# richarddurbin/hash10x

Measured on AMD Instinct MI355X. Metric: read-pairs/s through --readFQB + --hashDepthRange + --cluster (mosh construction + per-barcode clustering), higher is better.
Workload: dtype u64; 1 GPU; yeast-like-2.5M; read_pairs=2500000, barcodes=10000, B=24, k=21, w=31, clusterThreshold=5, parallelism=single GPU

## Files before the change

### hash10x_amd/csrc/common.hpp

```cpp
#pragma once
#include <hip/hip_runtime.h>
#include <cstdint>
#include <cstdio>
#include <cstdarg>
#include <cstring>
#include <cstdlib>
#include <ctime>
#include <string>
#include <vector>
#include <map>
#include <mutex>
#include "../../include/h10x.h"

namespace h10x {

constexpr int WAVE = 64;
typedef unsigned long long u64;
typedef uint32_t u32;
typedef uint16_t u16;
typedef uint8_t  u8;

static_assert(sizeof(h10x_block) == 32, "ClusterBlock layout (hash10x.c:62-70)");
static_assert(sizeof(h10x_clushash) == 8, "ClusterHash layout (hash10x.c:35-43)");

// ... 53 lines not shown
    if (!count) count = 1;
    size_t bytes = (count * sizeof(T) + 255) & ~(size_t)255;
    dev = AllocScope::device(); st = AllocScope::stream();
    hipError_t e = hipSuccess;
    void *q = DevCache::disabled() ? nullptr : DevCache::take(dev, st, bytes, cap);
    if (!q) {
      static const bool log = getenv("H10X_ALLOC_LOG") != nullptr;
      timespec t0, t1; if (log) clock_gettime(CLOCK_MONOTONIC, &t0);
      cap = bytes; e = hipMalloc(&q, bytes);
      if (e != hipSuccess && !DevCache::disabled()) { DevCache::trim(dev); e = hipMalloc(&q, bytes); }
      if (e == hipSuccess) { __atomic_fetch_add(&DevCache::freshCalls(), 1, __ATOMIC_RELAXED); __atomic_fetch_add(&DevCache::freshBytes(), (unsigned long long)bytes, __ATOMIC_RELAXED); }
      if (log) { clock_gettime(CLOCK_MONOTONIC, &t1); fprintf(stderr, "h10x alloc: %.1f MB fresh, %.3f ms\n", bytes / 1e6, (t1.tv_sec - t0.tv_sec) * 1e3 + (t1.tv_nsec - t0.tv_nsec) / 1e6); }
    }
    if (e == hipSuccess) { p = (T *)q; n = count; } else { p = nullptr; cap = 0; }
    if (e == hipSuccess && DevCache::poison()) (void)hipMemsetAsync(p, 0xA5, bytes, AllocScope::stream());
    return e;
  }
  void swap(DevBuf &o) { std::swap(p, o.p); std::swap(n, o.n); std::swap(cap, o.cap); std::swap(dev, o.dev); std::swap(st, o.st); }
  size_t bytes() const { return n * sizeof(T); }
};

enum TimerId { T_RUNS = 0, T_MOSH, T_FALLBACK, T_COMPACT, T_SORT_HASH, T_RANK, T_PROBE, T_CLUSHASH, T_CSR,
               T_GOOD, T_CLUSTER, T_CLUSTER_K, T_CLUSTER_MAIN, T_SPLIT, T_COUNT };
static const char *const kTimerNames[T_COUNT] = {
  "block_runs", "mosh_extract", "mosh_fallback", "compact_entries", "sort_by_hash", "index_rank",
  "probe_table", "clushash_build", "csr_build", "good_hashes", "cluster", "cluster_kernel", "cluster_main", "cluster_split" };

struct Timer { hipEvent_t a = nullptr, b = nullptr; double ms = 0; uint64_t launches = 0; bool pending = false; };

enum XchgId { X_HOST_COUNTS = 0, X_ENTRIES, X_FIRST_COUNTS, X_INDEX_BACK, X_INDEX_DEPTH, X_LIST_HEADS, X_LIST_DATA, X_TABLES, X_OWNER_LISTS, X_GATHER, X_COUNT };
static const char *const kXchgNames[X_COUNT] = {
  "host_counts (small host allgathers: sizes, counts)", "entries_to_hash_owners (all-to-all)", "first_seen_counts (allgather)", "indices_back (all-to-all)",
  "index_depth (allgather)", "list_heads (allgather: index + length of the in-range hashes)", "list_data (allgather: the in-range barcode lists)",
  "hash_tables (allgather: hashValue, for --writeHash / the crib)", "owner_lists_rebuild (after --clusterSplit)", "gather_to_rank0" };
struct XchgStat { u64 calls = 0, bytesOut = 0, bytesIn = 0, maxPeerOut = 0; Timer t, tIn; int beside = -1; };

constexpr size_t ROWS_PAD = 128;
constexpr int MAX_SEGS = 8;
struct BlockSeg { u32 localStart, count, globalBase; };
struct SegMap {
  int n; BlockSeg s[MAX_SEGS];
  __host__ __device__ u32 globalOf(u32 l) const {
    for (int k = n - 1; k > 0; --k) if (l >= s[k].localStart) return s[k].globalBase + (l - s[k].localStart);
    return s[0].globalBase + l;
  }
};
struct ShardSegInfo { u32 rank, localStart, count, globalBase; u64 entries; };

struct Ctx {
  h10x_params prm{};
  u64 keyInv = 1; int keyShift = 0; int keyBits = 64;
  bool wantPacked = false; int entCodeBits = 0;
  int device = 0;
  hipStream_t stream = nullptr;
  hipStream_t aux[3] = {nullptr, nullptr, nullptr};
  hipEvent_t evFork = nullptr, evJoin[3] = {nullptr, nullptr, nullptr};
  int numCU = 256;
  bool ownStream = false;
  std::string err;

  DevBuf<u32> hashIndex;
  DevBuf<u64> hashValue;
  DevBuf<u32> hashDepth;
  DevBuf<u64> rowStart;
  DevBuf<u32> rows;
  DevBuf<h10x_block> blocks;
  DevBuf<u64> blockOff;
  DevBuf<h10x_clushash> clusHash;
  u32 hashNumber = 1, nBlocks = 0;
  u32 maxBlockHashes = 0xFFFFFFFFu;
  u64 nEntries = 0, nRecords = 0;
  bool haveState = false;

  DevBuf<u8>  within;
  DevBuf<u16> goodPos;
  DevBuf<u32> nGood;
  DevBuf<u64> goodRow;
  DevBuf<u32> goodEntries;
  DevBuf<u32> clusterRaw;
  bool haveRange = false, haveGood = false; int rangeMin = 0, rangeMax = 0;
  u32 rangeHiMax = 0;
  u32 depthBound = 0xFFFFFFFFu;
  u32 maxGoodDepth = 0, maxGood = 0, meanGood = 0;

  DevBuf<u32> cribCount[2];
  DevBuf<u64> cribFirst[2];
  DevBuf<int16_t> cribChr; DevBuf<u16> cribPos; DevBuf<u8> cribType;
  DevBuf<u32> cribHist;
  u32 cribHistDim = 0; int cribGenomes = 0; bool haveCrib = false;

  struct Comm *comm = nullptr; bool sharded = false;
  u32 codeBase = 0, nBlocksGlobal = 0;
  SegMap segs{1, {{0, 0, 0}}};
  std::vector<ShardSegInfo> allSegs;
  u64 nEntriesGlobal = 0, nRecordsGlobal = 0;
  int rowShift = 0;
  bool ownerListsStale = false;
  DevBuf<u32> oRows, oSegStart, oIndex; u32 oU = 0; u64 oM = 0;
  DevBuf<u64> oHash;
  bool tablesPending = false;

  int64_t optMaxSlots = 0;
  int64_t optClusterLds = 0;
  int64_t optFirstGlobal = 0;
  int64_t optFirstCap = 0;
  int64_t optClusterThreads0 = 0, optClusterBudget0 = 0;
  int64_t optBigRanks = 0;
  int64_t optPrivTable = 0;
  int64_t optProbedTable = 0;
  int64_t optNoPack = 0;
  int64_t optNarrowFirst = 0;
  int64_t optTrEstDiv = 0;
  int64_t optTrClassT = -1;
  int64_t optTrPacked = -1;
  int64_t optStamps = 0;
  int64_t optChunk = 0;
  int64_t optChunkEof = 1;
  std::vector<u64> mergePoints; bool replayDone = false;
  int64_t optRowShift = -1;
  int64_t optReplySort = 0;
  int64_t optOverlap = 1;
  int64_t optOwnerCut = 0;
  int64_t optDeltaLists = -1;
  int64_t optRowsFakeBase = 0;
  int64_t optNbBudget = 0;
  u64 nbStats[4] = {0, 0, 0, 0};
  DevBuf<u32> ingestBuf; u64 ingestRecords = 0, ingestCap = 0; bool ingestAsync = false;
  static constexpr int INGEST_SLOTS = 8; hipEvent_t ingestEv[INGEST_SLOTS] = {};
  int64_t optFaultInject = 0;
  int faultAt(int region) { if (optFaultInject != region) return 0; optFaultInject = 0; return fail("injected fault in fork/join region %d", region); }
  bool timing = false;
  u32 *startFlags = nullptr;
  Timer timers[T_COUNT];
  XchgStat xs[X_COUNT];
  h10x_counters ctr{};

  int fail(const char *fmt, ...) {
    char buf[1024]; va_list ap; va_start(ap, fmt); vsnprintf(buf, sizeof buf, fmt, ap); va_end(ap);
    err = buf; return -1;
  }
  static constexpr size_t MAIL_BYTES = 4096, MAIL_ITEMS = 12;
  unsigned char *mail = nullptr; size_t mailUsed = 0; u32 mailSeq = 0; bool mailDirect = false;
  struct PendingRead { void *dst; const void *dev; size_t off, n; };
  std::vector<PendingRead> pendingReads;
  int readback(void *dst, const void *dev, size_t n) {
    if (!mail) {
      if (hipHostMalloc((void **)&mail, MAIL_BYTES + 64, hipHostMallocCoherent | hipHostMallocMapped) != hipSuccess) { mail = nullptr; return fail("hipHostMalloc of the read-back mailbox failed"); }
      memset(mail, 0, MAIL_BYTES + 64);
    }
    const size_t off = mailUsed, step = (n + 7) & ~(size_t)7;
    if (off + step > MAIL_BYTES || pendingReads.size() >= MAIL_ITEMS) {
      mailDirect = true;
      return hipMemcpyAsync(dst, dev, n, hipMemcpyDeviceToHost, stream) == hipSuccess ? 0 : fail("hipMemcpyAsync (device to host) failed");
    }
    mailUsed += step; pendingReads.push_back(PendingRead{dst, dev, off, n});
    return 0;
  }
  int syncReadbacks();
  int forkStreams(int n) {
    if (!evFork) {
      if (hipEventCreateWithFlags(&evFork, hipEventDisableTiming) != hipSuccess) return fail("hipEventCreate failed");
      for (int i = 0; i < 3; ++i) {
        if (hipStreamCreateWithFlags(&aux[i], hipStreamNonBlocking) != hipSuccess) return fail("hipStreamCreate failed");
        if (hipEventCreateWithFlags(&evJoin[i], hipEventDisableTiming) != hipSuccess) return fail("hipEventCreate failed");
      }
    }
// ... 179 lines not shown
```

### hash10x_amd/csrc/h10x_api.hip

```cpp
#include "common.hpp"
#include "comm.hpp"
#include "build_id.h"
#include <cstdlib>
#include <ctime>
#include <new>
#include <stdexcept>

using namespace h10x;

static int enter(Ctx &c) {
  if (hipSetDevice(c.device) != hipSuccess) return c.fail("hipSetDevice(%d) failed", c.device);
  AllocScope::stream() = c.stream; AllocScope::device() = c.device;
  DevCache::noteStream(c.device, c.stream);
  c.pendingReads.clear(); c.mailUsed = 0; c.mailDirect = false;
  c.stageReset();
  return 0;
}

struct h10x_ctx { Ctx c; };

extern "C" {

int h10x_abi_version(void) { return H10X_ABI_VERSION; }
const char *h10x_build_id(void) { return H10X_BUILD_ID; }
// ... 112 lines not shown
  if (!rm || !set) return -1;
  return rsGuard(M(set), [&] { return stageI_load(reinterpret_cast<RefMap **>(rm), M(set), index, offset, id, depth, rev, loc, max, nIds); });
}
void h10x_refmap_destroy(h10x_refmap *rm) { stageI_destroy(RM(rm)); }
const char *h10x_refmap_error(const h10x_refmap *rm) { return stageI_error(reinterpret_cast<const RefMap *>(rm)); }
int h10x_refmap_info(const h10x_refmap *rm, h10x_refmap_info_t *out) { if (!rm || !out) return -1; stageI_info(reinterpret_cast<const RefMap *>(rm), out); return 0; }
int h10x_refmap_add(h10x_refmap *rm, const uint8_t *codes, const uint64_t *seqStart, uint32_t nSeq, uint32_t idBase, uint64_t *nHits) {
  return rm ? rsGuard(stageI_set(RM(rm)), [&] { return stageI_add(RM(rm), codes, (const u64 *)seqStart, nSeq, idBase, (u64 *)nHits); }) : -1;
}
int h10x_refmap_pack(h10x_refmap *rm, uint32_t *n1, uint32_t *n2, uint32_t *nM) {
  return rm ? rsGuard(stageI_set(RM(rm)), [&] { return stageI_pack(RM(rm), n1, n2, nM); }) : -1;
}
int h10x_refmap_export(h10x_refmap *rm, const uint32_t **index, const uint32_t **offset, const uint32_t **id, const uint32_t **depth, const uint32_t **rev, const uint32_t **loc) {
  return rm ? stageI_export(RM(rm), index, offset, id, depth, rev, loc) : -1;
}
int h10x_refmap_query(h10x_refmap *rm, const uint8_t *codes, const uint64_t *seqStart, uint32_t nSeq, int wantSeeds) {
  return rm ? rsGuard(stageI_set(RM(rm)), [&] { return stageI_query(RM(rm), codes, (const u64 *)seqStart, nSeq, wantSeeds); }) : -1;
}
int h10x_refmap_results(h10x_refmap *rm, uint32_t *nQueries, const uint32_t **counts4, const uint64_t **recStart, const h10x_maprec_t **recs, const uint64_t **seedStart,
                        const h10x_mapseed_t **seeds, const uint32_t **seedPos) {
  return rm ? stageI_results(RM(rm), nQueries, counts4, (const u64 **)recStart, recs, (const u64 **)seedStart, seeds, seedPos) : -1;
}

static int create_fail(char *err, int errlen, const char *fmt, ...) {
  if (err && errlen > 0) { va_list ap; va_start(ap, fmt); vsnprintf(err, (size_t)errlen, fmt, ap); va_end(ap); }
  return -1;
}

int h10x_create(h10x_ctx **out, const h10x_params *p, int device, void *stream, char *err, int errlen) {
  if (!out || !p) return create_fail(err, errlen, "h10x_create: null argument");
  *out = nullptr;
  if (p->k <= 0 || p->w <= 0) return create_fail(err, errlen, "k %d, w %d must be > 0; run without args for usage", p->k, p->w);
  if (p->k >= 32) return create_fail(err, errlen, "seqhash k %d must be between 1 and 32\n", p->k);
  if (p->B < 20 || p->B > 30) return create_fail(err, errlen, "hashTableBits %d out of range 20-30", p->B);
  int n = 0;
  if (hipGetDeviceCount(&n) != hipSuccess || n <= 0)
    return create_fail(err, errlen, "no HIP device available: libh10x_hip has no CPU fallback");
  if (device < 0 || device >= n) return create_fail(err, errlen, "HIP device %d out of range 0..%d", device, n - 1);
  if (hipSetDevice(device) != hipSuccess) return create_fail(err, errlen, "hipSetDevice(%d) failed", device);
  static hipDeviceProp_t propCache[64]; static bool propOK[64];
  if (device >= 64) return create_fail(err, errlen, "HIP device %d out of range", device);
  if (!propOK[device]) {
    if (hipGetDeviceProperties(&propCache[device], device) != hipSuccess) return create_fail(err, errlen, "hipGetDeviceProperties failed");
    propOK[device] = true;
  }
  const hipDeviceProp_t &prop = propCache[device];
  if (strncmp(prop.gcnArchName, "gfx950", 6) != 0)
    return create_fail(err, errlen, "device %d is %s: this library is built for gfx950 (MI355X) only", device, prop.gcnArchName);
  h10x_ctx *h = new (std::nothrow) h10x_ctx();
  if (!h) return create_fail(err, errlen, "out of host memory");
  h->c.prm = *p; h->c.device = device; h->c.stream = (hipStream_t)stream; h->c.numCU = prop.multiProcessorCount;
  if (!stream) {
    if (hipStreamCreateWithFlags(&h->c.stream, hipStreamNonBlocking) != hipSuccess) { delete h; return create_fail(err, errlen, "hipStreamCreate failed"); }
    h->c.ownStream = true;
  }
  *out = h;
  return 0;
}

void h10x_destroy(h10x_ctx *h) {
  if (!h) return;
  (void)enter(h->c);
  (void)hipStreamSynchronize(h->c.stream);
  for (auto &t : h->c.timers) { if (t.a) (void)hipEventDestroy(t.a); if (t.b) (void)hipEventDestroy(t.b); }
  for (int i = 0; i < 3; ++i) { if (h->c.aux[i]) { (void)hipStreamSynchronize(h->c.aux[i]); (void)hipStreamDestroy(h->c.aux[i]); } if (h->c.evJoin[i]) (void)hipEventDestroy(h->c.evJoin[i]); }
  if (h->c.evFork) (void)hipEventDestroy(h->c.evFork);
  if (h->c.xStream) { (void)hipStreamSynchronize(h->c.xStream); (void)hipStreamDestroy(h->c.xStream); h->c.xStream = nullptr; }
  if (h->c.evXFork) (void)hipEventDestroy(h->c.evXFork);
  if (h->c.evXDone) (void)hipEventDestroy(h->c.evXDone);
  for (auto &e : h->c.ingestEv) if (e) (void)hipEventDestroy(e);
  if (h->c.startFlags) (void)hipHostFree(h->c.startFlags);
  if (h->c.mail) (void)hipHostFree(h->c.mail);
  hipStream_t own = h->c.ownStream ? h->c.stream : nullptr; const hipStream_t used = h->c.stream; const int dev = h->c.device;
  delete h;
  (void)hipStreamSynchronize(used);
  DevCache::retireStream(dev, used);
  if (own) (void)hipStreamDestroy(own);
}

const char *h10x_last_error(const h10x_ctx *h) { return h ? h->c.err.c_str() : "null context"; }

static void reset_state(Ctx &c) {
  c.haveState = false; c.haveRange = false; c.haveGood = false; c.rangeMin = c.rangeMax = 0; c.depthBound = 0xFFFFFFFFu; c.rangeHiMax = 0;
  c.within.release(); c.goodPos.release(); c.nGood.release(); c.goodEntries.release(); c.goodRow.release();
  c.hashIndex.release(); c.hashValue.release(); c.hashDepth.release(); c.rowStart.release(); c.rows.release();
  c.blocks.release(); c.blockOff.release(); c.clusHash.release(); c.clusterRaw.release();
  c.hashNumber = 1; c.nBlocks = 0; c.nEntries = 0; c.nRecords = 0; c.maxBlockHashes = 0xFFFFFFFFu;
  c.sharded = false; c.codeBase = 0; c.nBlocksGlobal = 0; c.oRows.release(); c.oSegStart.release(); c.oIndex.release(); c.oU = 0; c.oM = 0;
  c.oHash.release(); c.tablesPending = false;
  c.segs.n = 1; c.segs.s[0] = BlockSeg{0, 0, 0}; c.allSegs.clear(); c.nEntriesGlobal = c.nRecordsGlobal = 0; c.rowShift = 0; c.ownerListsStale = false;
  memset(&c.ctr, 0, sizeof c.ctr);
  c.haveCrib = false; c.cribGenomes = 0; c.cribChr.release(); c.cribPos.release(); c.cribType.release(); c.cribHist.release();
  for (int g = 0; g < 2; ++g) { c.cribCount[g].release(); c.cribFirst[g].release(); }
}

int h10x_read_fqb_device(h10x_ctx *h, const uint32_t *dRec, uint64_t n) {
  if (!h) return -1;
  Ctx &c = h->c;
  H10X_TRY(enter(c));
  if (n && !dRec) return c.fail("h10x_read_fqb_device: null records");
  reset_state(c);
  static const bool prof = getenv("H10X_HOSTPROF") != nullptr;
  timespec t0, t1, t2; clock_gettime(CLOCK_MONOTONIC, &t0);
  DevBuf<u64> entHash; DevBuf<u32> entCode, entRead;
  c.wantPacked = !c.optNoPack;
  { const int rcA = stageA_run(&c, dRec, n, entHash, entCode, entRead); c.wantPacked = false; if (rcA) return rcA; }
  c.segs.n = 1; c.segs.s[0] = BlockSeg{0, c.nBlocks, 0};
  clock_gettime(CLOCK_MONOTONIC, &t1);
  H10X_TRY(stageB_run(&c, entHash, entCode, entRead));
  clock_gettime(CLOCK_MONOTONIC, &t2);
  if (prof) fprintf(stderr, "hostprof: stageA %.3f ms, stageB %.3f ms (wall)\n", 1e3 * (t1.tv_sec - t0.tv_sec) + 1e-6 * (t1.tv_nsec - t0.tv_nsec),
                    1e3 * (t2.tv_sec - t1.tv_sec) + 1e-6 * (t2.tv_nsec - t1.tv_nsec));
  return 0;
}

int h10x_read_fqb(h10x_ctx *h, const uint32_t *hostRec, uint64_t n) {
  if (!h) return -1;
  Ctx &c = h->c;
  H10X_TRY(enter(c));
  if (n && !hostRec) return c.fail("h10x_read_fqb: null records");
  DevBuf<u32> d;
  H10X_HIP(&c, d.alloc(n * 30));
  if (n) H10X_HIP(&c, hipMemcpyAsync(d.p, hostRec, n * 120, hipMemcpyHostToDevice, c.stream));
  H10X_HIP(&c, hipStreamSynchronize(c.stream));
  return h10x_read_fqb_device(h, d.p, n);
}

__global__ void block_offsets_kernel(const h10x_block *__restrict__ blocks, u32 nBlocks, u32 *__restrict__ nHash) {
  const u32 i = blockIdx.x * blockDim.x + threadIdx.x;
  if (i <= nBlocks) nHash[i] = (i >= 1 && i < nBlocks) ? blocks[i].nHash : 0;
}

__global__ void validate_entries_kernel(const h10x_clushash *__restrict__ ch, const u64 *__restrict__ blockOff, const h10x_block *__restrict__ blocks, u32 nBlocks,
                                        u32 hashNumber, u32 *__restrict__ bad) {
  for (u32 b = blockIdx.x + 1; b < nBlocks; b += gridDim.x) {
    const u64 e0 = blockOff[b], e1 = blockOff[b + 1]; const u32 nSub = blocks[b].nSubCluster;
    if (threadIdx.x == 0 && nSub > 255) atomicAdd(&bad[2], 1u);
    for (u64 e = e0 + threadIdx.x; e < e1; e += blockDim.x) {
      const h10x_clushash x = ch[e];
      if (x.hash >= hashNumber) atomicAdd(&bad[0], 1u);
      if (x.subCluster > nSub) atomicAdd(&bad[3], 1u);
    }
  }
}
__global__ void validate_table_kernel(const u32 *__restrict__ table, u64 n, u32 hashNumber, u32 *__restrict__ bad) {
  u64 i = (u64)blockIdx.x * blockDim.x + threadIdx.x; const u64 stride = (u64)gridDim.x * blockDim.x;
  u32 mine = 0;
  for (; i < n; i += stride) if (table[i] >= hashNumber) ++mine;
  if (mine) atomicAdd(&bad[1], mine);
}

}

#include "prim.hpp"

extern "C" {

}
namespace h10x { int shard_adoptLoadedState(Ctx *c, Comm *cm, u32 codeBase, u32 nBlocksGlobal); }
static int upload_state(Ctx &c, const uint32_t *hashIndex, uint32_t hashNumber, const uint64_t *hashValue,
                        const uint32_t *hashDepth, const h10x_block *blocks, uint32_t nBlocks, const h10x_clushash *clusHash) {
  if (!hashIndex || !hashValue || !hashDepth || !blocks || nBlocks < 1 || hashNumber < 1) return c.fail("h10x_load_state: bad argument");
  reset_state(c);
  hipStream_t st = c.stream;
  const u64 tableSize = (u64)1 << c.prm.B;
  u64 H = 0;
  u32 maxHash = 0;
// ... 512 lines not shown
```

### hash10x_amd/csrc/prim.hip

```cpp
#include "prim.hpp"
#include <thread>
#include <rocprim/rocprim.hpp>

namespace h10x {

#define PRIM_TWO_PHASE(c, t, CALL)                                                               \
  do { size_t bytes = 0; void *tmp = nullptr;                                                    \
       hipError_t e = (CALL);                                                                    \
       if (e != hipSuccess) return (c)->fail("rocPRIM size query failed: %s", hipGetErrorName(e)); \
       if (bytes > (t).buf.n) { e = (t).buf.alloc(bytes + (bytes >> 2));                         \
         if (e != hipSuccess) return (c)->fail("out of device memory for %zu bytes of sort/scan scratch", bytes); } \
       tmp = (t).buf.p;                                                                          \
       e = (CALL);                                                                               \
       if (e != hipSuccess) return (c)->fail("rocPRIM call failed: %s", hipGetErrorName(e)); } while (0)

int prim_exclusive_scan_u32(Ctx *c, PrimTemp &t, const u32 *in, u32 *out, size_t n) {
  if (!n) return 0;
  PRIM_TWO_PHASE(c, t, rocprim::exclusive_scan(tmp, bytes, in, out, (u32)0, n, rocprim::plus<u32>(), c->stream));
  return 0;
}
struct RunHead {
  const u64 *key; size_t n; int cb;
  __device__ u32 operator()(size_t i) const { return (i < n && (i == 0 || (key[i] >> cb) != (key[i - 1] >> cb))) ? 1u : 0u; }
};
int prim_run_ordinals_u64(Ctx *c, PrimTemp &t, const u64 *key, int cb, u32 *ord, size_t n) {
  auto flags = rocprim::make_transform_iterator(rocprim::counting_iterator<size_t>(0), RunHead{key, n, cb});
  PRIM_TWO_PHASE(c, t, rocprim::exclusive_scan(tmp, bytes, flags, ord, (u32)0, n + 1, rocprim::plus<u32>(), c->stream));
  return 0;
}
int prim_exclusive_scan_u32_u64(Ctx *c, PrimTemp &t, const u32 *in, u64 *out, size_t n) {
  if (!n) return 0;
  auto in64 = rocprim::make_transform_iterator(in, [] __device__(u32 v) -> u64 { return (u64)v; });
  PRIM_TWO_PHASE(c, t, rocprim::exclusive_scan(tmp, bytes, in64, out, (u64)0, n, rocprim::plus<u64>(), c->stream));
  return 0;
}
int prim_inclusive_scan_u32(Ctx *c, PrimTemp &t, const u32 *in, u32 *out, size_t n) {
  if (!n) return 0;
  PRIM_TWO_PHASE(c, t, rocprim::inclusive_scan(tmp, bytes, in, out, n, rocprim::plus<u32>(), c->stream));
  return 0;
}
int prim_sort_pairs_u64_u32(Ctx *c, PrimTemp &t, const u64 *kin, u64 *kout, const u32 *vin, u32 *vout, size_t n, int b0, int b1) {
  if (!n) return 0;
  PRIM_TWO_PHASE(c, t, rocprim::radix_sort_pairs(tmp, bytes, kin, kout, vin, vout, n, (unsigned)b0, (unsigned)b1, c->stream));
  return 0;
}
int prim_sort_pairs_u32_u32(Ctx *c, PrimTemp &t, const u32 *kin, u32 *kout, const u32 *vin, u32 *vout, size_t n, int b0, int b1) {
  if (!n) return 0;
  PRIM_TWO_PHASE(c, t, rocprim::radix_sort_pairs(tmp, bytes, kin, kout, vin, vout, n, (unsigned)b0, (unsigned)b1, c->stream));
  return 0;
}
struct MailArgs { const unsigned char *src[Ctx::MAIL_ITEMS]; u32 off[Ctx::MAIL_ITEMS], n[Ctx::MAIL_ITEMS]; u32 count; };
__global__ void mail_post_kernel(MailArgs a, unsigned char *mail, u32 *flag, u32 seq) {
  for (u32 i = 0; i < a.count; ++i)
    for (u32 b = threadIdx.x; b < a.n[i]; b += blockDim.x) mail[a.off[i] + b] = a.src[i][b];
  __threadfence_system();
  __syncthreads();
  if (threadIdx.x == 0) __hip_atomic_store(flag, seq, __ATOMIC_RELEASE, __HIP_MEMORY_SCOPE_SYSTEM);
}
int Ctx::syncReadbacks() {
  hipError_t e = hipSuccess;
  if (pendingReads.empty() || mailDirect) e = hipStreamSynchronize(stream);
  if (!pendingReads.empty() && e == hipSuccess) {
    MailArgs a; a.count = (u32)pendingReads.size();
    for (u32 i = 0; i < a.count; ++i) { a.src[i] = (const unsigned char *)pendingReads[i].dev; a.off[i] = (u32)pendingReads[i].off; a.n[i] = (u32)pendingReads[i].n; }
    u32 *flag = (u32 *)(mail + MAIL_BYTES);
    const u32 seq = ++mailSeq ? mailSeq : ++mailSeq;
    mail_post_kernel<<<1, 64, 0, stream>>>(a, mail, flag, seq);
    e = hipGetLastError();
    for (u64 spins = 0; e == hipSuccess && __atomic_load_n(flag, __ATOMIC_ACQUIRE) != seq; ++spins) {
#if !defined(__HIP_DEVICE_COMPILE__)
#if defined(__x86_64__) || defined(__i386__)
      __builtin_ia32_pause();
#else
      std::this_thread::yield();
#endif
#endif
      if ((spins & 0xFFF) == 0xFFF) {
        const hipError_t q = hipStreamQuery(stream);
        if (q == hipErrorNotReady) continue;
        if (q == hipSuccess && __atomic_load_n(flag, __ATOMIC_ACQUIRE) == seq) break;
        e = q == hipSuccess ? hipErrorUnknown : q;
      }
    }
    if (e == hipSuccess) for (const PendingRead &r : pendingReads) memcpy(r.dst, mail + r.off, r.n);
  }
  pendingReads.clear(); mailUsed = 0; mailDirect = false;
  return e == hipSuccess ? 0 : fail("HIP error %s at a read-back", hipGetErrorString(e));
}

int prim_sort_pairs_u32_v16(Ctx *c, PrimTemp &t, const u32 *kin, u32 *kout, const Val16 *vin, Val16 *vout, size_t n, int b0, int b1) {
  if (!n) return 0;
  PRIM_TWO_PHASE(c, t, rocprim::radix_sort_pairs(tmp, bytes, kin, kout, vin, vout, n, (unsigned)b0, (unsigned)b1, c->stream));
  return 0;
}
using SortKeys64Config = rocprim::radix_sort_config<rocprim::default_config, rocprim::default_config,
    rocprim::radix_sort_onesweep_config<rocprim::kernel_config<1024, 8>, rocprim::kernel_config<1024, 8>, 8, rocprim::block_radix_rank_algorithm::match>, 1024 * 1024>;
int prim_sort_keys_u64(Ctx *c, PrimTemp &t, const u64 *kin, u64 *kout, size_t n, int b0, int b1) {
  if (!n) return 0;
  PRIM_TWO_PHASE(c, t, rocprim::radix_sort_keys<SortKeys64Config>(tmp, bytes, kin, kout, n, (unsigned)b0, (unsigned)(b1 > 64 ? 64 : b1), c->stream));
  return 0;
}
int prim_seg_sort_keys_u64(Ctx *c, PrimTemp &t, const u64 *kin, u64 *kout, u32 n, u32 nSeg, const u32 *begin, const u32 *end, int b0, int b1) {
  if (!n || !nSeg) return 0;
  PRIM_TWO_PHASE(c, t, rocprim::segmented_radix_sort_keys(tmp, bytes, kin, kout, n, nSeg, begin, end, (unsigned)b0, (unsigned)b1, c->stream));
  return 0;
}
int prim_seg_sort_keys_u32(Ctx *c, PrimTemp &t, const u32 *kin, u32 *kout, u32 n, u32 nSeg, const u32 *begin, const u32 *end, int b0, int b1) {
  if (!n || !nSeg) return 0;
  PRIM_TWO_PHASE(c, t, rocprim::segmented_radix_sort_keys(tmp, bytes, kin, kout, n, nSeg, begin, end, (unsigned)b0, (unsigned)b1, c->stream));
  return 0;
// ... 16 lines not shown
```

### hash10x_amd/csrc/prim.hpp

```cpp
#pragma once
#include "common.hpp"

namespace h10x {

struct PrimTemp { DevBuf<char> buf; };

int prim_run_ordinals_u64(Ctx *c, PrimTemp &t, const u64 *key, int cb, u32 *ord , size_t n);
int prim_exclusive_scan_u32(Ctx *c, PrimTemp &t, const u32 *in, u32 *out, size_t n);
int prim_exclusive_scan_u32_u64(Ctx *c, PrimTemp &t, const u32 *in, u64 *out, size_t n);
int prim_inclusive_scan_u32(Ctx *c, PrimTemp &t, const u32 *in, u32 *out, size_t n);
int prim_sort_pairs_u64_u32(Ctx *c, PrimTemp &t, const u64 *kin, u64 *kout, const u32 *vin, u32 *vout, size_t n, int beginBit, int endBit);
int prim_sort_pairs_u32_u32(Ctx *c, PrimTemp &t, const u32 *kin, u32 *kout, const u32 *vin, u32 *vout, size_t n, int beginBit, int endBit);
int prim_sort_keys_u64(Ctx *c, PrimTemp &t, const u64 *kin, u64 *kout, size_t n, int beginBit, int endBit);
struct Val16 { u64 a; u32 b, c; };
int prim_sort_pairs_u32_v16(Ctx *c, PrimTemp &t, const u32 *kin, u32 *kout, const Val16 *vin, Val16 *vout, size_t n, int beginBit, int endBit);
int prim_seg_sort_keys_u64(Ctx *c, PrimTemp &t, const u64 *kin, u64 *kout, u32 n, u32 nSeg, const u32 *begin, const u32 *end, int beginBit, int endBit);
int prim_seg_sort_keys_u32(Ctx *c, PrimTemp &t, const u32 *kin, u32 *kout, u32 n, u32 nSeg, const u32 *begin, const u32 *end, int beginBit, int endBit);
int prim_reduce_max_u32(Ctx *c, PrimTemp &t, const u32 *in, u32 *out, size_t n);
int prim_reduce_sum_u32_u64(Ctx *c, PrimTemp &t, const u32 *in, u64 *out, size_t n);

}
```

### hash10x_amd/csrc/stage_a.hip

```cpp
#include "common.hpp"
#include <algorithm>
#include "prim.hpp"

namespace h10x {

constexpr u64 EMPTY64 = ~0ULL;
constexpr u32 NHASH_OVERFLOW = 0xFFFFFFFFu;
constexpr int MOSH_THREADS = 256;
constexpr int REC_TILE = 16;
constexpr int SEQ_WORDS = 12;

struct MoshConst {
  int k, w, shift1;
  int n1, n2;
  int run;
  u64 factor1;
};
#define H10X_MOSH_DBG(bit) false

__device__ __forceinline__ u64 kmer_window(const u32 *seq, int p, int k) {
  const int wi = p >> 4, s = (p & 15) * 2;
  const u64 hi = ((u64)seq[wi] << 32) | (u64)seq[wi + 1];
  const u32 lo = seq[wi + 2];
  const u64 x = s ? ((hi << s) | (u64)(lo >> (32 - s))) : hi;
// ... 271 lines not shown
    }
  }
  while (qn) if (!queue_drain(table, mask, queue, qn, lane)) { sOverflow = 1; break; }
  __syncthreads();

  const u64 out0 = capOff[code];
  const u32 cap = S - (S >> 3);
  for (u32 base = 0; base < (H10X_MOSH_DBG(64) ? 0u : S); base += blockDim.x) {
    const u32 i = base + threadIdx.x;
    const u64 v = i < S ? table[i] : EMPTY64;
    const bool valid = !entry_empty(v);
    const u64 bal = __ballot(valid);
    const int lane = threadIdx.x & (WAVE - 1);
    u32 wbase = 0;
    if (lane == 0 && bal) wbase = atomicAdd(&sCount, (u32)__popcll(bal));
    wbase = __shfl(wbase, 0);
    if (valid) {
      const u32 pos = wbase + (u32)__popcll(bal & ((1ULL << lane) - 1));
      if (pos < cap) { stHash[out0 + pos] = mk64(hi32(v) >> 16, __builtin_amdgcn_alignbit(hi32(v), lo32(v), 16)); stRead[out0 + pos] = lo32(v) & 0xFFFFu; }
    }
  }
  __syncthreads();
  if (threadIdx.x == 0) {
    u32 n = sCount;
    if (sOverflow || n > cap) n = NHASH_OVERFLOW;
    else if (n == 0) { stHash[out0] = 0; stRead[out0] = 0; n = 1; }
    nHashOut[code] = n;
  }
}

template <bool W31>
__global__ __launch_bounds__(MOSH_THREADS)
void mosh_raw_kernel(const u32 *__restrict__ rec, u64 rec0, u32 nRead, MoshConst mc, u64 *__restrict__ rawKey, u32 *__restrict__ rawSlot) {
  __shared__ u32 tile[REC_TILE * 2 * SEQ_WORDS];
  const int nk = mc.n1 + mc.n2;
  for (u32 i = threadIdx.x; i < REC_TILE * 2 * SEQ_WORDS; i += blockDim.x) tile[i] = 0;
  for (u32 r0 = blockIdx.x * REC_TILE; r0 < nRead; r0 += gridDim.x * REC_TILE) {
    const int cnt = (int)min((u32)REC_TILE, nRead - r0);
    __syncthreads();
    stage_records(rec, rec0 + r0, cnt, tile);
    __syncthreads();
    for (int rr = 0; rr < cnt; ++rr)
      for (int t = threadIdx.x; t < nk; t += blockDim.x) {
        u64 h; const bool ok = mosh_of_slot<W31>(tile + rr * 2 * SEQ_WORDS, t, mc, h);
        const u64 slot = (u64)(r0 + rr) * nk + t;
        rawKey[slot] = ok ? h : EMPTY64;
        rawSlot[slot] = (u32)slot;
      }
  }
}

__global__ void unique_flags_kernel(const u64 *__restrict__ key, u64 n, u32 *__restrict__ flags) {
  u64 i = (u64)blockIdx.x * blockDim.x + threadIdx.x;
  const u64 stride = (u64)gridDim.x * blockDim.x;
  for (; i < n; i += stride) flags[i] = (key[i] != EMPTY64 && (i == 0 || key[i] != key[i - 1])) ? 1u : 0u;
}
__global__ void unique_scatter_kernel(const u64 *__restrict__ key, const u32 *__restrict__ slot, const u32 *__restrict__ flags,
                                      const u32 *__restrict__ pos, u64 n, u32 nk, u64 *__restrict__ outHash, u32 *__restrict__ outRead) {
  u64 i = (u64)blockIdx.x * blockDim.x + threadIdx.x;
  const u64 stride = (u64)gridDim.x * blockDim.x;
  for (; i < n; i += stride) if (flags[i]) { outHash[pos[i]] = key[i]; outRead[pos[i]] = slot[i] / nk; }
}

__global__ void set_nhash_kernel(h10x_block *__restrict__ blocks, const u32 *__restrict__ nHash, u32 nBlocks) {
  const u32 c = blockIdx.x * blockDim.x + threadIdx.x;
  if (c < nBlocks) blocks[c].nHash = nHash[c];
}

struct SrcPtr { const u64 *hash; const u32 *read; };
__global__ void count_overflow_kernel(const u32 *__restrict__ nHash, u32 nBlocks, u32 *__restrict__ count) {
  const u32 c = blockIdx.x * blockDim.x + threadIdx.x;
  const u64 bal = __ballot(c < nBlocks && nHash[c] == NHASH_OVERFLOW);
  if ((threadIdx.x & (WAVE - 1)) == 0 && bal) atomicAdd(count, (u32)__popcll(bal));
}

__global__ void compact_entries_kernel(const u64 *__restrict__ stHash, const u32 *__restrict__ stRead, const u64 *__restrict__ capOff,
                                       const SrcPtr *__restrict__ fb ,
                                       const u32 *__restrict__ nHash, const u64 *__restrict__ blockOff, u32 nBlocks,
                                       u64 keyInv, int keyShift, int codeBits ,
                                       u64 *__restrict__ entHash, u32 *__restrict__ entCode, u32 *__restrict__ entRead) {
  for (u32 c = blockIdx.x + 1; c < nBlocks; c += gridDim.x) {
    const u32 n = nHash[c]; if (!n) continue;
    const u64 *sh; const u32 *sr;
    if (fb[c].hash) { sh = fb[c].hash; sr = fb[c].read; } else { sh = stHash + capOff[c]; sr = stRead + capOff[c]; }
    const u64 o = blockOff[c];
    if (codeBits) for (u32 i = threadIdx.x; i < n; i += blockDim.x) { entHash[o + i] = (((sh[i] >> keyShift) * keyInv) << codeBits) | c; entRead[o + i] = sr[i]; }
    else for (u32 i = threadIdx.x; i < n; i += blockDim.x) { entHash[o + i] = (sh[i] >> keyShift) * keyInv; entCode[o + i] = c; entRead[o + i] = sr[i]; }
  }
}

__global__ void sort_keys_kernel(const u32 *__restrict__ rec, u64 n, u32 *__restrict__ key, u32 *__restrict__ idx) {
  u64 i = (u64)blockIdx.x * blockDim.x + threadIdx.x;
  const u64 stride = (u64)gridDim.x * blockDim.x;
  for (; i < n; i += stride) { key[i] = __builtin_bswap32(rec[i * 30]); idx[i] = (u32)i; }
}
__global__ void gather_records_kernel(const u32 *__restrict__ rec, const u32 *__restrict__ idx, u64 n, u32 *__restrict__ out) {
  u64 t = (u64)blockIdx.x * blockDim.x + threadIdx.x;
  const u64 stride = (u64)gridDim.x * blockDim.x, total = n * 30;
  for (; t < total; t += stride) { const u64 j = t / 30; const u32 w = (u32)(t - j * 30); out[t] = rec[(u64)idx[j] * 30 + w]; }
}
int stageA_sortRecords(Ctx *c, const u32 *dIn, u64 n, u32 *dOut) {
  hipStream_t st = c->stream; PrimTemp pt;
  if (n >= (1ULL << 32)) return c->fail("record sort: %llu records exceed this build's 2^32 limit", (u64)n);
  if (!n) return 0;
  DevBuf<u32> key, keyS, idx, idxS;
  H10X_HIP(c, key.alloc(n)); H10X_HIP(c, keyS.alloc(n)); H10X_HIP(c, idx.alloc(n)); H10X_HIP(c, idxS.alloc(n));
  const unsigned g = (unsigned)hmin<u64>(divUp(n, 256), 65535u * 4);
  sort_keys_kernel<<<g, 256, 0, st>>>(dIn, n, key.p, idx.p);
  H10X_TRY(prim_sort_pairs_u32_u32(c, pt, key.p, keyS.p, idx.p, idxS.p, n, 0, 32));
  gather_records_kernel<<<(unsigned)hmin<u64>(divUp(n * 30, 256), 65535u * 16), 256, 0, st>>>(dIn, idxS.p, n, dOut);
  H10X_HIP(c, hipGetLastError());
  H10X_HIP(c, hipStreamSynchronize(st));
  return 0;
}

int replayChunks(const std::vector<u64> &starts, const std::vector<u32> &zeroRuns, u64 chunk, std::vector<u64> &merges, bool eofPass) {
  merges.clear();
  const size_t R = starts.size() - 1; const u64 total = starts[R];
  if (!R || !total) return 0;
  std::vector<u32> zr(zeroRuns); std::sort(zr.begin(), zr.end());
  auto isZero = [&](size_t r) { return std::binary_search(zr.begin(), zr.end(), (u32)r); };
  auto runOf = [&](u64 pos) { return (size_t)(std::upper_bound(starts.begin(), starts.begin() + R, pos) - starts.begin()) - 1; };
  std::vector<size_t> swallowed;
  u64 pos = 0, head = 0; bool open = false, barcodeZero = true;
  while (pos < total) {
    const u64 carry = open ? pos - head : 0;
    if (chunk <= carry) return 1;
    if (barcodeZero && open) {
      const size_t r = runOf(pos);
      if (starts[r] == pos) { merges.push_back(pos); swallowed.push_back(r); }
    }
    if (!open) { head = pos; open = true; }
    const u64 end = head + chunk < total ? head + chunk : total;
    size_t q = runOf(end - 1);
    barcodeZero = isZero(q);
    while (std::binary_search(swallowed.begin(), swallowed.end(), q)) --q;
    head = starts[q];
    pos = end;
  }
  if (eofPass && open && total - head >= chunk) return 1;
  return 0;
}

int stageA_runStarts(Ctx *c, const u32 *dRec, u64 nRec, std::vector<u64> &starts, std::vector<u32> &zeroRuns) {
  hipStream_t st = c->stream; PrimTemp pt;
  starts.assign(1, 0); zeroRuns.clear();
  if (!nRec) return 0;
  DevBuf<u32> flags, code; DevBuf<u64> startRec;
  H10X_HIP(c, flags.alloc(nRec)); H10X_HIP(c, code.alloc(nRec));
  const unsigned g = (unsigned)hmin<u64>(divUp(nRec, 256), 65535u * 4);
  head_flags_kernel<<<g, 256, 0, st>>>(dRec, nRec, flags.p);
  H10X_TRY(prim_inclusive_scan_u32(c, pt, flags.p, code.p, nRec));
  u32 nRuns = 0;
  H10X_TRY(c->readback(&nRuns, code.p + (nRec - 1), 4));
  H10X_TRY(c->syncReadbacks());
  const u32 nBlocks = nRuns + 1;
  H10X_HIP(c, startRec.alloc((size_t)nBlocks + 1));
  block_starts_kernel<<<g, 256, 0, st>>>(flags.p, code.p, nRec, nBlocks, startRec.p);
  constexpr u32 ZCAP = 4096;
  DevBuf<u32> zl, zc; H10X_HIP(c, zl.alloc(ZCAP)); H10X_HIP(c, zc.alloc(1)); H10X_HIP(c, hipMemsetAsync(zc.p, 0, 4, st));
  zero_runs_kernel<<<divUp(nBlocks, 256), 256, 0, st>>>(dRec, startRec.p, nBlocks, zl.p, ZCAP, zc.p);
  starts.resize((size_t)nRuns + 1);
  H10X_HIP(c, hipMemcpyAsync(starts.data(), startRec.p + 1, ((size_t)nRuns + 1) * 8, hipMemcpyDeviceToHost, st));
  u32 nz = 0;
  H10X_TRY(c->readback(&nz, zc.p, 4));
  H10X_TRY(c->syncReadbacks());
  if (nz > ZCAP) return c->fail("%u separate runs of the all-A barcode: the input is not grouped by barcode", nz);
  zeroRuns.resize(nz);
  if (nz) { H10X_HIP(c, hipMemcpyAsync(zeroRuns.data(), zl.p, (size_t)nz * 4, hipMemcpyDeviceToHost, st)); H10X_HIP(c, hipStreamSynchronize(st)); }
  return 0;
}

int stageA_run(Ctx *c, const u32 *dRec, u64 nRec, DevBuf<u64> &entHash, DevBuf<u32> &entCode, DevBuf<u32> &entRead, bool hashLast, bool emptyIsNoBlock) {
  hipStream_t st = c->stream;
  PrimTemp pt;
  const int k = c->prm.k;
  MoshConst mc; mc.k = k; mc.w = c->prm.w; mc.shift1 = 64 - 2 * k; mc.factor1 = c->prm.factor1;
  mc.n1 = 127 - k + 1 > 0 ? 127 - k + 1 : 0;
  mc.n2 = 150 - k + 1 > 0 ? 150 - k + 1 : 0;
  mc.run = 8; while ((mc.n1 + mc.run - 1) / mc.run + (mc.n2 + mc.run - 1) / mc.run > 32) ++mc.run;
  const bool w31 = c->prm.w == 31;

  c->tstart(T_RUNS);
  u32 nBlocks = 2;
  DevBuf<u64> startRec;
  if (nRec) {
    DevBuf<u32> flags, code;
    H10X_HIP(c, flags.alloc(nRec)); H10X_HIP(c, code.alloc(nRec));
    const unsigned g = (unsigned)hmin<u64>(divUp(nRec, 256), 65535u * 4);
    if (c->optChunk > 0 && !c->replayDone) {
      std::vector<u64> starts; std::vector<u32> zeroRuns;
      H10X_TRY(stageA_runStarts(c, dRec, nRec, starts, zeroRuns));
      if (replayChunks(starts, zeroRuns, (u64)c->optChunk, c->mergePoints, c->optChunkEof != 0)) return c->fail("chunkSize too small");
    }
    c->replayDone = false;
    head_flags_kernel<<<g, 256, 0, st>>>(dRec, nRec, flags.p);
    if (!c->mergePoints.empty()) {
      DevBuf<u64> at; H10X_HIP(c, at.alloc(c->mergePoints.size()));
      H10X_HIP(c, hipMemcpyAsync(at.p, c->mergePoints.data(), c->mergePoints.size() * 8, hipMemcpyHostToDevice, st));
      clear_heads_kernel<<<divUp(c->mergePoints.size(), 256), 256, 0, st>>>(flags.p, at.p, (u32)c->mergePoints.size());
      H10X_HIP(c, hipStreamSynchronize(st));
      c->mergePoints.clear();
    }
    H10X_TRY(prim_inclusive_scan_u32(c, pt, flags.p, code.p, nRec));
    u32 nRuns = 0;
    H10X_TRY(c->readback(&nRuns, code.p + (nRec - 1), 4));
    H10X_TRY(c->syncReadbacks());
    nBlocks = nRuns + 1;
    H10X_HIP(c, startRec.alloc((size_t)nBlocks + 1));
    block_starts_kernel<<<g, 256, 0, st>>>(flags.p, code.p, nRec, nBlocks, startRec.p);
  } else {
    if (emptyIsNoBlock) nBlocks = 1;
    H10X_HIP(c, startRec.alloc(3));
    H10X_HIP(c, hipMemsetAsync(startRec.p, 0, 24, st));
  }
  c->nBlocks = nBlocks; c->nRecords = nRec;
  H10X_HIP(c, c->blocks.alloc(nBlocks));

  u32 maxSlots = 16384;
  if (c->optMaxSlots > 0) maxSlots = (u32)c->optMaxSlots;
  const int packedOK = (2 * k + 16 <= 64) ? 1 : 0;
  DevBuf<u32> slots, list0, list1, list2, listF, counts, nHash;
  H10X_HIP(c, slots.alloc(nBlocks)); H10X_HIP(c, list0.alloc(nBlocks)); H10X_HIP(c, list1.alloc(nBlocks)); H10X_HIP(c, list2.alloc(nBlocks));
  H10X_HIP(c, listF.alloc(nBlocks)); H10X_HIP(c, counts.alloc(4)); H10X_HIP(c, nHash.alloc((size_t)nBlocks + 1));
  H10X_HIP(c, hipMemsetAsync(counts.p, 0, 16, st));
  H10X_HIP(c, hipMemsetAsync(nHash.p, 0, ((size_t)nBlocks + 1) * 4, st));
  classify_kernel<<<divUp(nBlocks, 256), 256, 0, st>>>(startRec.p, nBlocks, c->blocks.p, slots.p, maxSlots, packedOK,
                                                      list0.p, list1.p, list2.p, listF.p, counts.p, hashLast ? 1 : 0);
  DevBuf<u64> capOff; H10X_HIP(c, capOff.alloc((size_t)nBlocks + 1));
  H10X_TRY(prim_exclusive_scan_u32_u64(c, pt, slots.p, capOff.p, nBlocks));
  u32 hc[4]; u64 capTotal = 0; u32 lastSlots = 0;
  H10X_TRY(c->readback(hc, counts.p, 16));
  H10X_TRY(c->readback(&capTotal, capOff.p + (nBlocks - 1), 8));
  H10X_TRY(c->readback(&lastSlots, slots.p + (nBlocks - 1), 4));
  H10X_TRY(c->syncReadbacks());
  capTotal += lastSlots;
  c->tstop(T_RUNS);

  DevBuf<u64> stHash; DevBuf<u32> stRead;
  H10X_HIP(c, stHash.alloc(capTotal)); H10X_HIP(c, stRead.alloc(capTotal));
  c->tstart(T_MOSH);
  ForkGuard forkGuard(c);
  H10X_TRY(c->forkStreams(2));
#define H10X_MOSH_LAUNCH(W, LL, FK, TH, STREAM)                                                                                    \
    { if (lds > 48 * 1024) H10X_HIP(c, hipFuncSetAttribute((const void *)mosh_lds_kernel<W, LL, FK>, hipFuncAttributeMaxDynamicSharedMemorySize, (int)lds)); \
      mosh_lds_kernel<W, LL, FK><<<n, TH, lds, STREAM>>>(dRec, list, n, startRec.p, slots.p, capOff.p, mc, (u32)tableBytes, stHash.p, stRead.p, nHash.p); }
#define H10X_MOSH_CLASS(TH, STREAM)                                                                                                \
    { if (fastK && w31) H10X_MOSH_LAUNCH(true, 8, true, TH, STREAM) else if (fastK) H10X_MOSH_LAUNCH(false, 8, true, TH, STREAM)   \
      else if (w31 && mc.run == 8) H10X_MOSH_LAUNCH(true, 8, false, TH, STREAM) else if (w31) H10X_MOSH_LAUNCH(true, 9, false, TH, STREAM) \
      else if (mc.run == 8) H10X_MOSH_LAUNCH(false, 8, false, TH, STREAM) else H10X_MOSH_LAUNCH(false, 9, false, TH, STREAM) }
  const bool fastK = k >= 17 && k <= 30 && mc.run == 8;
  for (int cls = 2; cls >= 0; --cls) {
    const u32 n = hc[cls]; if (!n) continue;
    const u32 *list = cls == 0 ? list0.p : cls == 1 ? list1.p : list2.p;
    const size_t tableBytes = (size_t)hmin<u32>(4096u << cls, maxSlots) * 8;
    const size_t lds = tableBytes + (size_t)((cls == 2 ? 1024 : 512) / WAVE) * MOSH_QCAP * 8;
    if (cls == 2) H10X_MOSH_CLASS(1024, c->aux[0]) else if (cls == 1) H10X_MOSH_CLASS(512, c->aux[1]) else H10X_MOSH_CLASS(512, st)
    H10X_HIP(c, hipGetLastError());
  }
#undef H10X_MOSH_CLASS
#undef H10X_MOSH_LAUNCH
  H10X_TRY(c->faultAt(1));
  H10X_TRY(c->joinStreams(2));
  forkGuard.done();
  c->tstop(T_MOSH);

  DevBuf<u32> nOverflow; H10X_HIP(c, nOverflow.alloc(1)); H10X_HIP(c, hipMemsetAsync(nOverflow.p, 0, 4, st));
  count_overflow_kernel<<<divUp(nBlocks, 256), 256, 0, st>>>(nHash.p, nBlocks, nOverflow.p);
  H10X_HIP(c, c->blockOff.alloc((size_t)nBlocks + 1));
  H10X_TRY(prim_exclusive_scan_u32_u64(c, pt, nHash.p, c->blockOff.p, (size_t)nBlocks + 1));
  u64 H = 0, lastStart = 0; u32 hOverflow = 0, hMaxHash = 0xFFFFFFFFu;
  DevBuf<u32> dMaxHash; H10X_HIP(c, dMaxHash.alloc(1));
  H10X_TRY(prim_reduce_max_u32(c, pt, nHash.p, dMaxHash.p, nBlocks));
  H10X_TRY(c->readback(&hMaxHash, dMaxHash.p, 4));
  H10X_TRY(c->readback(&H, c->blockOff.p + nBlocks, 8));
  H10X_TRY(c->readback(&lastStart, startRec.p + (nBlocks - 1), 8));
  H10X_TRY(c->readback(&hOverflow, nOverflow.p, 4));
  H10X_TRY(c->syncReadbacks());
  const bool anyFallback = hc[3] || hOverflow;
  std::vector<u32> hNHash, hListF(hc[3]);
  std::vector<u64> hStart;
  if (anyFallback) {
    hNHash.resize(nBlocks + 1); hStart.resize(nBlocks + 1);
    H10X_HIP(c, hipMemcpyAsync(hNHash.data(), nHash.p, (size_t)nBlocks * 4, hipMemcpyDeviceToHost, st));
    H10X_HIP(c, hipMemcpyAsync(hStart.data(), startRec.p, ((size_t)nBlocks + 1) * 8, hipMemcpyDeviceToHost, st));
    if (hc[3]) H10X_HIP(c, hipMemcpyAsync(hListF.data(), listF.p, (size_t)hc[3] * 4, hipMemcpyDeviceToHost, st));
    H10X_HIP(c, hipStreamSynchronize(st));
    for (u32 b = 1; b + (hashLast ? 0 : 1) < nBlocks; ++b) if (hNHash[b] == NHASH_OVERFLOW) hListF.push_back(b);
  }
  std::vector<SrcPtr> hFb;
  std::vector<DevBuf<u64> *> keepH; std::vector<DevBuf<u32> *> keepR;
  c->ctr.fallback_blocks = hListF.size();
  if (!hListF.empty()) {
    hFb.assign(nBlocks, SrcPtr{nullptr, nullptr});
    c->tstart(T_FALLBACK);
    const u32 nk = (u32)(mc.n1 + mc.n2);
    for (u32 b : hListF) {
      const u32 nr = (u32)(hStart[b + 1] - hStart[b]);
      const u64 nSlot = (u64)nr * nk;
      DevBuf<u64> *oh = new DevBuf<u64>(); DevBuf<u32> *orr = new DevBuf<u32>(); keepH.push_back(oh); keepR.push_back(orr);
      u32 nUniq = 0;
      if (nSlot >= (1ULL << 32)) return c->fail("barcode block %u too large for the global mosh path (%llu k-mer slots)", b, (u64)nSlot);
      if (nSlot) {
        DevBuf<u64> k0, k1; DevBuf<u32> v0, v1, fl, ps;
        H10X_HIP(c, k0.alloc(nSlot)); H10X_HIP(c, k1.alloc(nSlot)); H10X_HIP(c, v0.alloc(nSlot)); H10X_HIP(c, v1.alloc(nSlot));
        H10X_HIP(c, fl.alloc(nSlot + 1)); H10X_HIP(c, ps.alloc(nSlot + 1));
        const unsigned g = (unsigned)hmin<u64>(divUp(nr, REC_TILE), 4096);
        if (w31) mosh_raw_kernel<true><<<g, MOSH_THREADS, 0, st>>>(dRec, hStart[b], nr, mc, k0.p, v0.p);
        else     mosh_raw_kernel<false><<<g, MOSH_THREADS, 0, st>>>(dRec, hStart[b], nr, mc, k0.p, v0.p);
        H10X_TRY(prim_sort_pairs_u64_u32(c, pt, k0.p, k1.p, v0.p, v1.p, nSlot, 0, 64));
        const unsigned g2 = (unsigned)hmin<u64>(divUp(nSlot, 256), 65535);
        unique_flags_kernel<<<g2, 256, 0, st>>>(k1.p, nSlot, fl.p);
        H10X_HIP(c, hipMemsetAsync(fl.p + nSlot, 0, 4, st));
        H10X_TRY(prim_exclusive_scan_u32(c, pt, fl.p, ps.p, nSlot + 1));
        H10X_HIP(c, hipMemcpyAsync(&nUniq, ps.p + nSlot, 4, hipMemcpyDeviceToHost, st));
        H10X_HIP(c, hipStreamSynchronize(st));
        H10X_HIP(c, oh->alloc(nUniq ? nUniq : 1)); H10X_HIP(c, orr->alloc(nUniq ? nUniq : 1));
        if (nUniq) unique_scatter_kernel<<<g2, 256, 0, st>>>(k1.p, v1.p, fl.p, ps.p, nSlot, nk, oh->p, orr->p);
        H10X_HIP(c, hipStreamSynchronize(st));
      } else { H10X_HIP(c, oh->alloc(1)); H10X_HIP(c, orr->alloc(1)); }
      if (!nUniq) {
        H10X_HIP(c, hipMemsetAsync(oh->p, 0, 8, st)); H10X_HIP(c, hipMemsetAsync(orr->p, 0, 4, st)); nUniq = 1;
      }
      hNHash[b] = nUniq; hFb[b] = SrcPtr{oh->p, orr->p};
    }
    H10X_HIP(c, hipMemcpyAsync(nHash.p, hNHash.data(), (size_t)nBlocks * 4, hipMemcpyHostToDevice, st));
    c->tstop(T_FALLBACK);
  }

  c->tstart(T_COMPACT);
  DevBuf<SrcPtr> dFb; H10X_HIP(c, dFb.alloc(nBlocks));
  if (hFb.empty()) H10X_HIP(c, hipMemsetAsync(dFb.p, 0, (size_t)nBlocks * sizeof(SrcPtr), st));
  else {
    H10X_HIP(c, hipMemcpyAsync(dFb.p, hFb.data(), (size_t)nBlocks * sizeof(SrcPtr), hipMemcpyHostToDevice, st));
    H10X_TRY(prim_exclusive_scan_u32_u64(c, pt, nHash.p, c->blockOff.p, (size_t)nBlocks + 1));
    H10X_HIP(c, hipMemcpyAsync(&H, c->blockOff.p + nBlocks, 8, hipMemcpyDeviceToHost, st));
    H10X_HIP(c, hipStreamSynchronize(st));
  }
  if (H >= (1ULL << 32)) return c->fail("%llu (barcode,hash) entries exceed this build's 2^32 per-GPU limit", (u64)H);
  c->nEntries = H;
  if (!hNHash.empty()) { hMaxHash = 0; for (u32 b = 0; b < nBlocks; ++b) hMaxHash = hNHash[b] > hMaxHash ? hNHash[b] : hMaxHash; }
  c->maxBlockHashes = hMaxHash;
  set_nhash_kernel<<<divUp(nBlocks, 256), 256, 0, st>>>(c->blocks.p, nHash.p, nBlocks);
  H10X_HIP(c, entHash.alloc(H)); H10X_HIP(c, entRead.alloc(H));
  {
    u64 m = (u64)c->prm.w; int s = 0; while (!(m & 1)) { m >>= 1; ++s; }
    u64 inv = m; for (int it = 0; it < 6; ++it) inv *= 2 - m * inv;
    const int k2 = 2 * c->prm.k; const u64 maxH = k2 >= 64 ? ~0ULL : ((u64)1 << k2) - 1, maxQ = maxH / (u64)c->prm.w;
    int b = 1; while (b < 64 && (maxQ >> b)) ++b;
    c->keyInv = inv; c->keyShift = s; c->keyBits = b;
    int cb = 1; while (cb < 32 && ((nBlocks - 1) >> cb)) ++cb;
    c->entCodeBits = (c->wantPacked && b + cb <= 63) ? cb : 0;
  }
  if (!c->entCodeBits) H10X_HIP(c, entCode.alloc(H));
  if (H) compact_entries_kernel<<<hmin<u32>(nBlocks, 8192), 256, 0, st>>>(stHash.p, stRead.p, capOff.p, dFb.p, nHash.p, c->blockOff.p, nBlocks,
                                                                        c->keyInv, c->keyShift, c->entCodeBits, entHash.p, entCode.p, entRead.p);
  H10X_HIP(c, hipGetLastError());
  if (!hFb.empty()) H10X_HIP(c, hipStreamSynchronize(st));
  c->tstop(T_COMPACT);
  for (auto *p : keepH) delete p;
  for (auto *p : keepR) delete p;

  u64 hashedPairs = hashLast ? nRec : (nBlocks >= 2 ? lastStart : 0);
  c->ctr.pairs = nRec; c->ctr.kmers = hashedPairs * (u64)(mc.n1 + mc.n2); c->ctr.entries = H;
  return 0;
}

__global__ void warm_stageA_kernel() {}
void warm_stageA(hipStream_t st) { warm_stageA_kernel<<<1, 1, 0, st>>>(); }

}
```

### hash10x_amd/csrc/stage_b.hip

```cpp
#include "common.hpp"
#include "prim.hpp"
#include <rocprim/block/block_radix_sort.hpp>

namespace h10x {

constexpr u32 SLOT_EMPTY = 0xFFFFFFFFu;
static int bitsFor(u64 maxValue) { int b = 1; while (b < 64 && (maxValue >> b)) ++b; return b; }

__global__ void seg_scatter_kernel(const u64 *__restrict__ sHash, const u32 *__restrict__ sCode,
                                   const u32 *__restrict__ ord, u64 n, u64 *__restrict__ dHash, u32 *__restrict__ dFirst,
                                   u32 *__restrict__ segStart, u32 *__restrict__ iota) {
  u64 i = (u64)blockIdx.x * blockDim.x + threadIdx.x;
  const u64 stride = (u64)gridDim.x * blockDim.x;
  for (; i < n; i += stride) if (ord[i + 1] != ord[i]) {
    const u32 d = ord[i];
    dHash[d] = sHash[i]; dFirst[d] = sCode[i]; segStart[d] = (u32)i; iota[d] = d;
  }
}
__global__ void seg_scatter_packed_kernel(const u64 *__restrict__ sKey, int cb,
                                          const u32 *__restrict__ ord, u64 n, Val16 *__restrict__ dVal, u32 *__restrict__ dFirst, u32 *__restrict__ rows) {
  u64 i = (u64)blockIdx.x * blockDim.x + threadIdx.x;
  const u64 stride = (u64)gridDim.x * blockDim.x;
  const u64 cmask = ((u64)1 << cb) - 1;
  for (; i < n; i += stride) {
    const u64 k = sKey[i]; const u32 code = (u32)(k & cmask);
    rows[i] = code;
    const u32 d = ord[i], d1 = ord[i + 1];
    if (d1 != d) { dVal[d].a = k >> cb; dVal[d].b = (u32)i; dFirst[d] = code; }
    if (i + 1 == n || ord[i + 2] != d1) dVal[d1 - 1].c = (u32)i + 1;
  }
}
__global__ void assign_index_v16_kernel(const Val16 *__restrict__ val, u32 U, u64 w , u64 *__restrict__ hashValue, u32 *__restrict__ hashDepth,
                                        u64 *__restrict__ rowStart) {
  const u32 i = blockIdx.x * blockDim.x + threadIdx.x;
  if (i == 0) { hashValue[0] = 0; hashDepth[0] = 0; rowStart[0] = 0; }
  if (i >= U) return;
  const Val16 v = val[i];
  hashValue[i + 1] = v.a * w; hashDepth[i + 1] = v.c - v.b; rowStart[i + 1] = v.b;
}

__global__ void assign_index_kernel(const u32 *__restrict__ order, const u64 *__restrict__ dHash, const u32 *__restrict__ segStart,
                                    u32 U, u64 w , u64 *__restrict__ hashValue, u32 *__restrict__ hashDepth, u64 *__restrict__ rowStart) {
  const u32 i = blockIdx.x * blockDim.x + threadIdx.x;
  if (i == 0) { hashValue[0] = 0; hashDepth[0] = 0; rowStart[0] = 0; }
  if (i >= U) return;
  const u32 d = order[i];
  hashValue[i + 1] = dHash[d] * w;
  hashDepth[i + 1] = segStart[d + 1] - segStart[d];
  rowStart[i + 1] = segStart[d];
}

__global__ void probe_insert_kernel(const u64 *__restrict__ hashValue, u32 hashNumber, int B, u32 *__restrict__ table) {
  const u32 first = blockIdx.x * blockDim.x + threadIdx.x + 1;
  const u64 mask = ((u64)1 << B) - 1;
  for (u32 start = first; start < hashNumber; start += gridDim.x * blockDim.x) {
    u32 cur = start;
    u64 h = hashValue[cur];
    u64 slot = h & mask, step = ((h >> B) & mask) | 1;
    for (;;) {
      const u32 old = atomicMin(&table[slot], cur);
      if (old == SLOT_EMPTY) break;
      if (old > cur) {
        cur = old; h = hashValue[cur]; step = ((h >> B) & mask) | 1;
      }
      slot = (slot + step) & mask;
    }
  }
}
__global__ void probe_finish_kernel(u32 *__restrict__ table, u64 n) {
  u64 i = (u64)blockIdx.x * blockDim.x + threadIdx.x;
  const u64 stride = (u64)gridDim.x * blockDim.x;
  for (; i < n; i += stride) if (table[i] == SLOT_EMPTY) table[i] = 0;
}

constexpr u64 SLOT_EMPTY64 = ~0ULL;
__global__ void probe_insert64_kernel(const u64 *__restrict__ hashValue, u32 hashNumber, int B, u64 w, int qBits, u64 *__restrict__ table) {
  const u32 first = blockIdx.x * blockDim.x + threadIdx.x + 1;
  const u64 mask = ((u64)1 << B) - 1, qmask = ((u64)1 << qBits) - 1;
  for (u32 start = first; start < hashNumber; start += gridDim.x * blockDim.x) {
    u64 h = hashValue[start];
    u64 cur = ((u64)start << qBits) | (h / w);
    u64 slot = h & mask, step = ((h >> B) & mask) | 1;
    for (;;) {
      const u64 old = atomicMin((unsigned long long *)&table[slot], (unsigned long long)cur);
      if (old == SLOT_EMPTY64) break;
      if (old > cur) {
        cur = old; h = (old & qmask) * w; step = ((h >> B) & mask) | 1;
      }
      slot = (slot + step) & mask;
    }
  }
}
__global__ void probe_insertP_kernel(const u64 *__restrict__ hashValue, u32 hashNumber, int B, int SH, int PB, u64 *__restrict__ table, u32 *__restrict__ fail) {
  const u32 first = blockIdx.x * blockDim.x + threadIdx.x + 1;
  const u64 mask = ((u64)1 << B) - 1, pmask = ((u64)1 << PB) - 1, umask = ((u64)1 << (SH - PB)) - 1;
  for (u32 start = first; start < hashNumber; start += gridDim.x * blockDim.x) {
    const u64 h = hashValue[start];
    u64 cur = ((u64)start << SH) | ((h >> B) << PB);
    u64 slot = h & mask, step = ((h >> B) & mask) | 1;
    for (;;) {
      const u64 old = atomicMin((unsigned long long *)&table[slot], (unsigned long long)cur);
      if (old == SLOT_EMPTY64) break;
      if (old > cur) { cur = old; step = (((cur >> PB) & umask) & mask) | 1; }
      if ((cur & pmask) == pmask) { *fail = 1; break; }
      ++cur;
      slot = (slot + step) & mask;
    }
  }
}
__global__ void probe_finish64_kernel(const u64 *__restrict__ table64, u64 n, int qBits, u32 *__restrict__ table) {
  u64 i = (u64)blockIdx.x * blockDim.x + threadIdx.x;
  const u64 stride = (u64)gridDim.x * blockDim.x;
// ... 203 lines not shown
          if (j < IPT) {
            const u32 e = (u32)j * THREADS + threadIdx.x;
            u32 kk;
            if (privT) kk = priv_find(table64, privT, q[j], hashIndex, hashValue, B, w, t[g]);
            else {
              const u64 h = q[j] * w; u64 slot = h & mask; const u64 step = ((h >> B) & mask) | 1;
              u64 tt = t[g];
              if (probeBits) { u64 want = (h >> B) << probeBits; while (tt != SLOT_EMPTY64 && (tt & qmask) != want) { slot = (slot + step) & mask; ++want; tt = table64[slot]; } }
              else while (tt != SLOT_EMPTY64 && (tt & qmask) != q[j]) { slot = (slot + step) & mask; tt = table64[slot]; }
              kk = tt == SLOT_EMPTY64 ? 0u : (u32)(tt >> qBits);
            }
            k[j] = e < n ? kk : 0xFFFFFFFFu;
          }
        }
      }
    } else if (replyPos) {
      u32 pp[IPT];
#pragma unroll
      for (int j = 0; j < IPT; ++j) { const u32 e = (u32)j * THREADS + threadIdx.x; pp[j] = replyPos[o + (e < n ? e : n - 1)]; }
#pragma unroll
      for (int j = 0; j < IPT; ++j) { const u32 e = (u32)j * THREADS + threadIdx.x; v[j] = entRead[o + (e < n ? e : n - 1)] & 0xFFFFu; }
#pragma unroll
      for (int j = 0; j < IPT; ++j) { const u32 e = (u32)j * THREADS + threadIdx.x; const u32 kk = replyIdx[pp[j]]; k[j] = e < n ? kk : 0xFFFFFFFFu; }
    } else {
#pragma unroll
      for (int j = 0; j < IPT; ++j) {
        const u32 e = (u32)j * THREADS + threadIdx.x;
        k[j] = 0xFFFFFFFFu; v[j] = 0;
        if (e < n) { const u64 t = key[o + e]; k[j] = (u32)(t >> 32); v[j] = (u32)t & 0xFFFFu; }
      }
    }
    __syncthreads();
    Sort::sort(k, v, n, storage);
#pragma unroll
    for (int j = 0; j < IPT; ++j) {
      const u32 e = (u32)j * THREADS + threadIdx.x;
      if (e < n) { h10x_clushash r; r.hash = k[j]; r.read = (u16)v[j]; r.subCluster = 0; r.flags = 0; out[o + e] = r; }
    }
  }
}

static int clusHashByBlocks(Ctx *c, const u64 *entHash, const u32 *entRead, const u64 *key, const u64 *table64, int privT = 0, const u32 *replyIdx = nullptr, const u32 *replyPos = nullptr,
                            int probeSH = 0, int probeBits = 0 ) {
  hipStream_t st = c->stream; const u32 nBlocks = c->nBlocks;
  H10X_HIP(c, c->clusHash.alloc(c->nEntries));
  if (!c->nEntries || nBlocks < 2) return 0;
  int sortBits = bitsFor(c->hashNumber) + 1 > 32 ? 32 : bitsFor(c->hashNumber) + 1;
  const int B = c->prm.B; const u64 w = (u64)c->prm.w; const int qBits = probeBits ? probeSH : c->keyBits;
  DevBuf<u32> lists, counts;
  H10X_TRY(stageB_blockClassLists(c, lists, counts));
  const unsigned gridBig = hmin<u32>(nBlocks, (u32)c->numCU * 8), gridSmall = hmin<u32>(nBlocks, 65535u * 4);
#define H10X_CH_LAUNCH(T, I, LOOK, CLS, STREAM) clushash_block_kernel<T, I, LOOK><<<(CLS == 0 ? gridSmall : gridBig), T, 0, STREAM>>>(entHash, entRead, key, c->blockOff.p, \
    lists.p + (size_t)CLS * nBlocks, counts.p + CLS, table64, B, w, qBits, (key || replyPos) ? 0 : c->entCodeBits, sortBits, c->clusHash.p, privT, c->hashIndex.p, c->hashValue.p, replyIdx, replyPos, probeBits)
  const int side = c->maxBlockHashes > BLOCK_SORT_CAP1 ? 2 : (c->maxBlockHashes > BLOCK_SORT_CAP0 ? 1 : 0);
  ForkGuard forkGuard(c);
  if (side) H10X_TRY(c->forkStreams(side));
  if (key || replyPos) { H10X_CH_LAUNCH(H10X_BS_T0, H10X_BS_I0, false, 0, st); if (side >= 1) H10X_CH_LAUNCH(H10X_BS_T1, H10X_BS_I1, false, 1, c->aux[0]); if (side >= 2) H10X_CH_LAUNCH(1024, 8, false, 2, c->aux[1]); }
  else { H10X_CH_LAUNCH(H10X_BS_T0, H10X_BS_I0, true, 0, st); if (side >= 1) H10X_CH_LAUNCH(H10X_BS_T1, H10X_BS_I1, true, 1, c->aux[0]); if (side >= 2) H10X_CH_LAUNCH(1024, 8, true, 2, c->aux[1]); }
#undef H10X_CH_LAUNCH
  H10X_TRY(c->faultAt(2));
  if (side) H10X_TRY(c->joinStreams(side));
  forkGuard.done();
  H10X_HIP(c, hipGetLastError());
  return 0;
}

int stageB_run(Ctx *c, DevBuf<u64> &entHash, DevBuf<u32> &entCode, DevBuf<u32> &entRead) {
  hipStream_t st = c->stream; PrimTemp pt;
  const u64 H = c->nEntries; const int B = c->prm.B; const u32 nBlocks = c->nBlocks;
  const unsigned gH = (unsigned)hmin<u64>(divUp(H ? H : 1, 256), 65535u * 2);
  const u64 tableSize = (u64)1 << B;

  c->tstart(T_SORT_HASH);
  DevBuf<u64> sHash; DevBuf<u32> sCode;
  const int cb = c->entCodeBits;
  H10X_HIP(c, sHash.alloc(H)); H10X_HIP(c, sCode.alloc(H + ROWS_PAD));
  if (cb) H10X_TRY(prim_sort_keys_u64(c, pt, entHash.p, sHash.p, H, cb, cb + c->keyBits));
  else H10X_TRY(prim_sort_pairs_u64_u32(c, pt, entHash.p, sHash.p, entCode.p, sCode.p, H, 0, c->keyBits));
  c->tstop(T_SORT_HASH);

  c->tstart(T_RANK);
  u32 U = 0;
  DevBuf<u64> dHash; DevBuf<u32> dFirst, segStart, iota, order, dFirstSorted; DevBuf<Val16> dVal, dValSorted;
  {
    DevBuf<u32> ord;
    H10X_HIP(c, ord.alloc(H + 2));
    H10X_TRY(prim_run_ordinals_u64(c, pt, sHash.p, cb, ord.p, H));
    H10X_TRY(c->readback(&U, ord.p + H, 4));
    H10X_TRY(c->syncReadbacks());
    if ((u64)U + 1 > (tableSize >> 2) - 2) return c->fail("hashTableSize is too small");
    H10X_HIP(c, dFirst.alloc(U)); H10X_HIP(c, dFirstSorted.alloc(U));
    if (cb) { H10X_HIP(c, dVal.alloc(U)); H10X_HIP(c, dValSorted.alloc(U)); }
    else { H10X_HIP(c, dHash.alloc(U)); H10X_HIP(c, segStart.alloc((size_t)U + 1)); H10X_HIP(c, iota.alloc(U)); H10X_HIP(c, order.alloc(U)); }
    if (H && cb) seg_scatter_packed_kernel<<<gH, 256, 0, st>>>(sHash.p, cb, ord.p, H, dVal.p, dFirst.p, sCode.p);
    else if (H) {
      seg_scatter_kernel<<<gH, 256, 0, st>>>(sHash.p, sCode.p, ord.p, H, dHash.p, dFirst.p, segStart.p, iota.p);
      H10X_HIP(c, hipMemsetD32Async((hipDeviceptr_t)(segStart.p + U), (int)(u32)H, 1, st));
    }
  }
  c->hashNumber = U + 1; c->depthBound = nBlocks;
  H10X_HIP(c, c->hashValue.alloc((size_t)U + 1)); H10X_HIP(c, c->hashDepth.alloc((size_t)U + 1));
  H10X_HIP(c, c->rowStart.alloc((size_t)U + 2));
  if (cb) {
    H10X_TRY(prim_sort_pairs_u32_v16(c, pt, dFirst.p, dFirstSorted.p, dVal.p, dValSorted.p, U, 0, bitsFor(nBlocks)));
    assign_index_v16_kernel<<<divUp((u64)U + 1, 256), 256, 0, st>>>(dValSorted.p, U, (u64)c->prm.w, c->hashValue.p, c->hashDepth.p, c->rowStart.p);
  } else {
    H10X_TRY(prim_sort_pairs_u32_u32(c, pt, dFirst.p, dFirstSorted.p, iota.p, order.p, U, 0, bitsFor(nBlocks)));
    assign_index_kernel<<<divUp((u64)U + 1, 256), 256, 0, st>>>(order.p, dHash.p, segStart.p, U, (u64)c->prm.w, c->hashValue.p, c->hashDepth.p, c->rowStart.p);
  }
  c->rows.swap(sCode);
  c->tstop(T_RANK);
  sHash.release(); dHash.release(); dFirst.release(); iota.release(); dFirstSorted.release(); dVal.release(); dValSorted.release();

  const bool forcePriv = (c->optPrivTable == 1 || c->optPrivTable == 3) && c->keyBits <= 40;
  const bool wideTable = !forcePriv && c->keyBits + (B - 2) <= 64 && c->keyBits < 64;
  DevBuf<u64> table64;
  const int hashBits = 2 * c->prm.k, UB = hashBits > B ? hashBits - B : 0, PBroom = 64 - (B - 2) - UB;
  int PB = 0, SH = 0; bool probed = false;
  if (!forcePriv && c->optProbedTable != 2 && (!wideTable || c->optProbedTable == 1 || c->optProbedTable == 3) && PBroom >= 12 && c->keyBits < 64) {
    PB = PBroom > 24 ? 24 : PBroom; if (c->optProbedTable == 3) PB = 1;
    SH = UB + PB;
    c->tstart(T_PROBE);
    DevBuf<u32> failFlag; u32 failed = 0;
    H10X_HIP(c, table64.alloc(tableSize)); H10X_HIP(c, c->hashIndex.alloc(tableSize)); H10X_HIP(c, failFlag.alloc(1));
    H10X_HIP(c, hipMemsetAsync(table64.p, 0xFF, tableSize * 8, st)); H10X_HIP(c, hipMemsetAsync(failFlag.p, 0, 4, st));
    if (U) probe_insertP_kernel<<<hmin<u32>(divUp(U, 256), 16384), 256, 0, st>>>(c->hashValue.p, U + 1, B, SH, PB, table64.p, failFlag.p);
    H10X_TRY(c->readback(&failed, failFlag.p, 4));
    H10X_TRY(c->syncReadbacks());
    probed = !failed;
    if (probed) probe_finish64_kernel<<<(unsigned)hmin<u64>(divUp(tableSize, 256), 65535u * 2), 256, 0, st>>>(table64.p, tableSize, SH, c->hashIndex.p);
    else { table64.release(); c->hashIndex.release(); }
    c->tstop(T_PROBE);
    c->ctr.index_table_form = probed ? 2 : 3;
  }
  if (probed) {}
  else if (wideTable) {
    if (c->ctr.index_table_form != 3) c->ctr.index_table_form = 1;
    c->tstart(T_PROBE);
    H10X_HIP(c, table64.alloc(tableSize)); H10X_HIP(c, c->hashIndex.alloc(tableSize));
    H10X_HIP(c, hipMemsetAsync(table64.p, 0xFF, tableSize * 8, st));
    if (U) probe_insert64_kernel<<<hmin<u32>(divUp(U, 256), 16384), 256, 0, st>>>(c->hashValue.p, U + 1, B, (u64)c->prm.w, c->keyBits, table64.p);
    probe_finish64_kernel<<<(unsigned)hmin<u64>(divUp(tableSize, 256), 65535u * 2), 256, 0, st>>>(table64.p, tableSize, c->keyBits, c->hashIndex.p);
    c->tstop(T_PROBE);
  } else { if (c->ctr.index_table_form != 3) c->ctr.index_table_form = 0; H10X_TRY(stageB_buildProbeTable(c)); }

  c->tstart(T_CLUSHASH);
  if (H && probed && c->maxBlockHashes <= BLOCK_SORT_MAX) {
    H10X_TRY(clusHashByBlocks(c, entHash.p, entRead.p, nullptr, table64.p, 0, nullptr, nullptr, SH, PB));
    table64.release();
  } else if (H && !probed && wideTable && c->maxBlockHashes <= BLOCK_SORT_MAX) {
    H10X_TRY(clusHashByBlocks(c, entHash.p, entRead.p, nullptr, table64.p));
    table64.release();
  } else if (H && !probed && !wideTable && c->maxBlockHashes <= BLOCK_SORT_MAX && c->keyBits <= 40 && c->optPrivTable != 2) {
    int T = 16; while (((u64)1 << T) < 2 * ((u64)U + 1) && T < 32) ++T;
    if (c->optPrivTable == 3) { T = 4; while (((u64)1 << T) < ((u64)U + 1) / 2 && T < 32) ++T; }
    if (T < c->keyBits - 24) T = c->keyBits - 24;
    DevBuf<u64> priv;
    H10X_HIP(c, priv.alloc((size_t)1 << T));
    H10X_HIP(c, hipMemsetAsync(priv.p, 0xFF, ((size_t)1 << T) * 8, st));
    if (U) priv_insert_kernel<<<hmin<u32>(divUp(U, 256), 16384), 256, 0, st>>>(c->hashValue.p, U + 1, (u64)c->prm.w, T, priv.p);
    H10X_TRY(clusHashByBlocks(c, entHash.p, entRead.p, nullptr, priv.p, T));
  } else if (H) {
    DevBuf<u64> key; H10X_HIP(c, key.alloc(H));
    if (wideTable && !probed) lookup_pack64_kernel<<<gH, 256, 0, st>>>(entHash.p, entRead.p, H, table64.p, B, (u64)c->prm.w, c->keyBits, cb, key.p);
    else lookup_pack_kernel<<<gH, 256, 0, st>>>(entHash.p, entRead.p, H, c->hashIndex.p, c->hashValue.p, B, (u64)c->prm.w, cb, key.p);
    table64.release();
    H10X_TRY(stageB_finishClusHash(c, key));
  } else H10X_HIP(c, c->clusHash.alloc(0));
  c->tstop(T_CLUSHASH);
  c->ctr.distinct = U;
  c->haveState = true;
  return 0;
}

int stageB_buildProbeTable(Ctx *c) {
  hipStream_t st = c->stream; const int B = c->prm.B; const u64 tableSize = (u64)1 << B; const u32 U = c->hashNumber - 1;
  c->tstart(T_PROBE);
  H10X_HIP(c, c->hashIndex.alloc(tableSize));
// ... 74 lines not shown
```

### hash10x_amd/csrc/stage_c.hip

```cpp
#include "common.hpp"
#include <chrono>
#include "prim.hpp"
#include <type_traits>
#include <rocprim/block/block_radix_sort.hpp>

namespace h10x {


constexpr int CL_THREADS_SMALL = 1024;
constexpr int CL_THREADS_HUGE = 1024;
constexpr u16 NONE16 = 0xFFFF;
constexpr u32 NOHANDLE = 0xFFFFFFFFu;
constexpr int ROWS_IN_FLIGHT = 4;
constexpr int RCHUNK = 4;

__global__ void within_kernel(const u32 *__restrict__ depth, u32 hashNumber, int lo, int hi, u8 *__restrict__ within) {
  const u32 i = blockIdx.x * blockDim.x + threadIdx.x;
  if (i >= hashNumber) return;
  const int n = (int)depth[i];
  if (n >= lo && n < hi) within[i] = 1;
}
__global__ void within_depth_kernel(const u32 *__restrict__ depth, const u8 *__restrict__ within, u32 hashNumber, u32 *__restrict__ out,
                                    const u64 *__restrict__ rowStart, u32 rowShift, u64 *__restrict__ rowInfo ) {
  const u32 i = blockIdx.x * blockDim.x + threadIdx.x;
  if (i < hashNumber) {
    const u32 wd = within[i] ? depth[i] + 1 : 0;
    out[i] = wd; if (rowInfo) rowInfo[i] = (u64)(u32)(rowStart[i] >> rowShift) | ((u64)wd << 32);
  }
}

template <typename KT>
__global__ __launch_bounds__(256)
void good_keys_kernel(const h10x_clushash *__restrict__ ch, const u64 *__restrict__ blockOff, const h10x_block *__restrict__ blocks,
                      u32 nBlocks, const u32 *__restrict__ wdepth ,
                      KT *__restrict__ key, u32 *__restrict__ nGood, u32 *__restrict__ segEnd, u32 *__restrict__ entries ) {
  __shared__ u32 sCount; __shared__ unsigned long long sDepth;
  for (u32 c = blockIdx.x; c < nBlocks; c += gridDim.x) {
    const u64 o = blockOff[c]; const u32 nHash = blocks[c].nHash;
    __syncthreads();
    if (threadIdx.x == 0) { sCount = 0; sDepth = 0; }
    __syncthreads();
    unsigned long long myDepth = 0;
    if (nHash <= 65535) {
      for (u32 base = 0; base < nHash; base += blockDim.x) {
        const u32 p = base + threadIdx.x;
        u32 wd = 0; bool good = false;
        if (p < nHash) { wd = wdepth[ch[o + p].hash]; good = wd != 0; if (good) myDepth += wd - 1; }
        const u64 bal = __ballot(good);
        const int lane = threadIdx.x & (WAVE - 1);
        u32 wb = 0;
        if (lane == 0 && bal) wb = atomicAdd(&sCount, (u32)__popcll(bal));
        wb = __shfl(wb, 0);
        if (good) key[o + wb + (u32)__popcll(bal & ((1ULL << lane) - 1))] = (KT)(((KT)(wd - 1) << 16) | (KT)p);
      }
    }
    for (int sft = 32; sft; sft >>= 1) myDepth += __shfl_down(myDepth, sft);
    if ((threadIdx.x & (WAVE - 1)) == 0 && myDepth) atomicAdd(&sDepth, myDepth);
    __syncthreads();
    if (threadIdx.x == 0) { nGood[c] = sCount; segEnd[c] = (u32)o + sCount; entries[c] = sDepth > 0xFFFFFFFFull ? 0xFFFFFFFFu : (u32)sDepth; }
  }
}
template <typename KT>
__global__ void good_pos_kernel(const KT *__restrict__ key, u64 n, u16 *__restrict__ pos) {
  u64 i = (u64)blockIdx.x * blockDim.x + threadIdx.x;
  const u64 stride = (u64)gridDim.x * blockDim.x;
  for (; i < n; i += stride) pos[i] = (u16)(key[i] & 0xFFFF);
}
__global__ void offsets32c_kernel(const u64 *__restrict__ off, u32 n, u32 *__restrict__ out) {
  const u32 i = blockIdx.x * blockDim.x + threadIdx.x;
  if (i < n) out[i] = (u32)off[i];
}

template <int THREADS, int IPT>
__global__ __launch_bounds__(THREADS)
void good_block_kernel(const h10x_clushash *__restrict__ ch, const u64 *__restrict__ blockOff, const h10x_block *__restrict__ blocks,
                       const u32 *__restrict__ list, const u32 *__restrict__ count ,
                       const u64 *__restrict__ rowInfo , int sortBits,
                       u16 *__restrict__ goodPos, u32 *__restrict__ nGood, u32 *__restrict__ entries ,
                       u64 *__restrict__ goodRow ) {
  using Sort = rocprim::block_radix_sort<u32, THREADS, IPT, u64>;
  __shared__ typename Sort::storage_type storage;
  __shared__ u32 sCount; __shared__ unsigned long long sDepth;
  const u32 nList = *count;
  for (u32 wi = blockIdx.x; wi < nList; wi += gridDim.x) {
    const u32 c = list[wi];
    const u32 nHash = blocks[c].nHash;
    const u64 o = blockOff[c];
    __syncthreads();
    if (threadIdx.x == 0) { sCount = 0; sDepth = 0; }
    __syncthreads();
    u32 k[IPT]; u64 v[IPT]; u32 mine = 0; unsigned long long myDepth = 0;
#pragma unroll
    for (int j = 0; j < IPT; ++j) { k[j] = 0xFFFFFFFFu; v[j] = threadIdx.x * IPT + (u32)j; }
    if (nHash) {
      u32 hs[IPT]; u64 ri[IPT];
#pragma unroll
      for (int j = 0; j < IPT; ++j) { const u32 p = threadIdx.x * IPT + (u32)j; hs[j] = ch[o + (p < nHash ? p : nHash - 1)].hash; }
#pragma unroll
      for (int j = 0; j < IPT; ++j) ri[j] = rowInfo[hs[j]];
#pragma unroll
      for (int j = 0; j < IPT; ++j) {
        const u32 p = threadIdx.x * IPT + (u32)j; const u32 wd = (u32)(ri[j] >> 32);
        if (p < nHash && wd) { k[j] = wd - 1; ++mine; myDepth += wd - 1; v[j] = (u64)p | ((ri[j] & 0xFFFFFFFFull) << 16); }
      }
    }
    for (int sft = 32; sft; sft >>= 1) { mine += (u32)__shfl_down((int)mine, sft); myDepth += __shfl_down(myDepth, sft); }
    if ((threadIdx.x & (WAVE - 1)) == 0 && mine) { atomicAdd(&sCount, mine); atomicAdd(&sDepth, myDepth); }
    Sort().sort_to_striped(k, v, storage, 0, sortBits);
    __syncthreads();
    const u32 nG = sCount;
#pragma unroll
    for (int j = 0; j < IPT; ++j) {
      const u32 e = (u32)j * THREADS + threadIdx.x;
      if (e < nG) {
        goodPos[o + e] = (u16)v[j];
        goodRow[o + e] = (u64)(u32)(v[j] >> 16) | ((u64)k[j] << 32);
      }
    }
    if (threadIdx.x == 0) { nGood[c] = nG; entries[c] = sDepth > 0xFFFFFFFFull ? 0xFFFFFFFFu : (u32)sDepth; }
  }
}

__global__ void good_rows_kernel(const h10x_clushash *__restrict__ ch, const u64 *__restrict__ blockOff, const u32 *__restrict__ nGood, const u16 *__restrict__ goodPos, u32 nBlocks,
                                 const u32 *__restrict__ hashDepth, const u64 *__restrict__ rowStart, u32 rowShift, u64 *__restrict__ goodRow);
static int bitsForC(u64 maxValue) { int b = 1; while (b < 64 && (maxValue >> b)) ++b; return b; }

int stageC_depthRange(Ctx *c, int lo, int hi) {
  hipStream_t st = c->stream; PrimTemp pt;
  if (!c->haveState) return c->fail("no hash state loaded: use readFQB or readHash first");
  c->haveGood = false;
  c->tstart(T_GOOD);
  const u32 U1 = c->hashNumber; const u32 nBlocks = c->nBlocks; const u64 H = c->nEntries;
  if (!(c->haveRange && lo == c->rangeMin && hi == c->rangeMax)) {
    if (!c->haveRange) { H10X_HIP(c, c->within.alloc(U1)); H10X_HIP(c, hipMemsetAsync(c->within.p, 0, U1, st)); }
    within_kernel<<<divUp(U1, 256), 256, 0, st>>>(c->hashDepth.p, U1, lo, hi, c->within.p);
    c->haveRange = true; c->rangeMin = lo; c->rangeMax = hi;
    if (hi > 0 && (u32)hi > c->rangeHiMax) c->rangeHiMax = (u32)hi;
  }
  XGuard xGuard(c);
  if (c->sharded) { c->tstop(T_GOOD); H10X_TRY(shard_exchangeRows(c)); c->tstart(T_GOOD); }
  DevBuf<u64> key, keyS; DevBuf<u32> key32, keyS32, off32, segEnd, wdepth, red;
  H10X_HIP(c, off32.alloc((size_t)nBlocks + 1));
  H10X_HIP(c, segEnd.alloc(nBlocks)); H10X_HIP(c, wdepth.alloc(U1)); H10X_HIP(c, red.alloc(2));
  H10X_HIP(c, c->nGood.alloc(nBlocks)); H10X_HIP(c, c->goodPos.alloc(H)); H10X_HIP(c, c->goodEntries.alloc(nBlocks)); H10X_HIP(c, c->goodRow.alloc(H));
  const u32 goodDepthBound = hmin<u32>(c->depthBound, c->rangeHiMax ? c->rangeHiMax - 1 : 0);
  const bool narrow = goodDepthBound <= 65535u;
  const bool byBlocks = narrow && c->maxBlockHashes <= BLOCK_SORT_MAX;
  DevBuf<u64> rowInfo; if (byBlocks) H10X_HIP(c, rowInfo.alloc(U1));
  within_depth_kernel<<<divUp(U1, 256), 256, 0, st>>>(c->hashDepth.p, c->within.p, U1, wdepth.p, c->rowStart.p, (u32)c->rowShift, rowInfo.p);
  H10X_TRY(prim_reduce_max_u32(c, pt, wdepth.p, red.p, U1));
  if (byBlocks) {
    int db = 1; while (db < 16 && (goodDepthBound >> db)) ++db;
    const int sortBits = db + 1;
    DevBuf<u32> lists, counts;
    H10X_TRY(stageB_blockClassLists(c, lists, counts));
    const unsigned gridBig = hmin<u32>(nBlocks, (u32)c->numCU * 8), gridSmall = hmin<u32>(nBlocks, 65535u * 4);
    const int side = c->maxBlockHashes > BLOCK_SORT_CAP1 ? 2 : (c->maxBlockHashes > BLOCK_SORT_CAP0 ? 1 : 0);
    ForkGuard forkGuard(c);
    if (side) H10X_TRY(c->forkStreams(side));
#define H10X_GOOD_LAUNCH(T, I, CLS, STREAM)                                                                                         \
    { const u32 *const L = lists.p + (size_t)CLS * nBlocks, *const N = counts.p + CLS; const unsigned grid = CLS == 0 ? gridSmall : gridBig; \
      good_block_kernel<T, I><<<grid, T, 0, STREAM>>>(c->clusHash.p, c->blockOff.p, c->blocks.p, L, N, rowInfo.p, sortBits, c->goodPos.p, c->nGood.p, c->goodEntries.p, c->goodRow.p); }
    H10X_GOOD_LAUNCH(H10X_BS_T0, H10X_BS_I0, 0, st)
    if (side >= 1) H10X_GOOD_LAUNCH(H10X_BS_T1, H10X_BS_I1, 1, c->aux[0])
    if (side >= 2) H10X_GOOD_LAUNCH(1024, 8, 2, c->aux[1])
#undef H10X_GOOD_LAUNCH
    H10X_TRY(c->faultAt(3));
    if (side) H10X_TRY(c->joinStreams(side));
    forkGuard.done();
  }
  else if (narrow) { H10X_HIP(c, key32.alloc(H)); H10X_HIP(c, keyS32.alloc(H)); } else { H10X_HIP(c, key.alloc(H)); H10X_HIP(c, keyS.alloc(H)); }
  if (byBlocks) {}
  else if (narrow) good_keys_kernel<u32><<<hmin<u32>(nBlocks, 16384), 256, 0, st>>>(c->clusHash.p, c->blockOff.p, c->blocks.p, nBlocks, wdepth.p,
                                                                             key32.p, c->nGood.p, segEnd.p, c->goodEntries.p);
  else good_keys_kernel<u64><<<hmin<u32>(nBlocks, 16384), 256, 0, st>>>(c->clusHash.p, c->blockOff.p, c->blocks.p, nBlocks, wdepth.p,
                                                                      key.p, c->nGood.p, segEnd.p, c->goodEntries.p);
  H10X_TRY(prim_reduce_max_u32(c, pt, c->nGood.p, red.p + 1, nBlocks));
  DevBuf<u64> redSum; H10X_HIP(c, redSum.alloc(1));
  H10X_TRY(prim_reduce_sum_u32_u64(c, pt, c->nGood.p, redSum.p, nBlocks));
  u32 hr[2]; u64 sumGood = 0;
  H10X_TRY(c->readback(hr, red.p, 8));
  H10X_TRY(c->readback(&sumGood, redSum.p, 8));
  H10X_TRY(c->syncReadbacks());
  hr[0] = hr[0] ? hr[0] - 1 : 0;
  c->maxGoodDepth = hr[0]; c->maxGood = hr[1]; c->meanGood = nBlocks > 1 ? (u32)(sumGood / (nBlocks - 1)) : 0;
  offsets32c_kernel<<<divUp((u64)nBlocks + 1, 256), 256, 0, st>>>(c->blockOff.p, nBlocks + 1, off32.p);
  if (H && !byBlocks) {
    if (narrow) {
      H10X_TRY(prim_seg_sort_keys_u32(c, pt, key32.p, keyS32.p, (u32)H, nBlocks, off32.p, segEnd.p, 0, 16 + bitsForC(hr[0])));
      good_pos_kernel<u32><<<(unsigned)hmin<u64>(divUp(H, 256), 65535u * 2), 256, 0, st>>>(keyS32.p, H, c->goodPos.p);
    } else {
      H10X_TRY(prim_seg_sort_keys_u64(c, pt, key.p, keyS.p, (u32)H, nBlocks, off32.p, segEnd.p, 0, 16 + bitsForC(hr[0])));
      good_pos_kernel<u64><<<(unsigned)hmin<u64>(divUp(H, 256), 65535u * 2), 256, 0, st>>>(keyS.p, H, c->goodPos.p);
    }
  }
  if (!byBlocks && nBlocks) good_rows_kernel<<<hmin<u32>(nBlocks, 65535u * 4), 256, 0, st>>>(c->clusHash.p, c->blockOff.p, c->nGood.p, c->goodPos.p, nBlocks, c->hashDepth.p, c->rowStart.p,
                                                                                           (u32)c->rowShift, c->goodRow.p);
  H10X_HIP(c, hipGetLastError());
  H10X_TRY(c->xJoin());
  c->haveGood = true;
  c->tstop(T_GOOD);
  return 0;
}

struct ClusterArgs {
  h10x_block *blocks; const u64 *blockOff; h10x_clushash *clusHash;
  const u16 *goodPos; const u32 *nGood;
  const u64 *goodRow;
  const u32 *rows;
  const u32 *list; u32 nList; u32 *workCounter;
  u32 *started;
  const u32 *front; u32 nFront;
  u32 nBlocks; int threshold;
  SegMap segs;
  u32 rowShift;
  u32 nBlocksFirst;
  u32 firstCap;
  u32 hashMinSlots;
  u32 hashBits;
  u16 *handles; size_t handleStride; u32 hStride;
  const u32 *entries;
  u32 *overflow, *overflowCount;
  unsigned char *scratch; size_t scratchStride;
  u32 maxGood;
  u32 ldsBudget;
  u64 *res;
  u64 *stats;
  u64 *phase;
  u32 narrowFirst;
  u32 tpClassT;
};

#define RES_PACK(best, q, tot) ((u64)(best) | ((u64)(q) << 16) | ((u64)(tot) << 40))
constexpr u32 RES_COUNT_MAX = (1u << 24) - 1;
struct Work {
  u16 *first;
  u32 *bm; u16 *pre;
  u16 *root;
  u32 *hist;
  u32 histWords;
};
__host__ __device__ inline size_t pad16(size_t b) { return (b + 15) & ~(size_t)15; }
__host__ __device__ inline size_t workBytes(u32 nFirst, u32 n, u32 nWaves, u32 bmWords) {
  size_t b = pad16((size_t)nFirst * 2) + pad16((size_t)bmWords * 4) + pad16((size_t)bmWords * 2);
  b += pad16((size_t)n * 2);
  b += (size_t)nWaves * (((size_t)n + 3) / 4) * 4;
  return b + 16;
}
constexpr u32 MIN_HIST_WAVES = 5;
constexpr u32 RANKED_FIRST_PER_RANK = 6;
__host__ __device__ inline u32 rankedFirstEstimate(u32 nBarcodes, u32 n) { const u64 e = (u64)RANKED_FIRST_PER_RANK * n; return e < nBarcodes ? (u32)e : nBarcodes; }
__host__ __device__ inline u32 rankedFirstEstimateE(u32 nBarcodes, u32 n, u32 entries, u32 div = 7) { const u32 a = rankedFirstEstimate(nBarcodes, n), b = entries / div; const u32 m = a > b ? a : b; return m < nBarcodes ? m : nBarcodes; }
__host__ __device__ inline u32 histWaves(u32 nFirst, u32 n, u32 maxWaves, u32 bmWords, size_t budget) {
  const size_t fixed = workBytes(nFirst, n, 0, bmWords), per = (((size_t)n + 3) / 4) * 4;
  if (fixed + MIN_HIST_WAVES * per > budget) return 0;
  const size_t wv = (budget - fixed) / (per ? per : 1);
  return wv < maxWaves ? (u32)wv : maxWaves;
}
__device__ inline Work carve(unsigned char *base, u32 nFirst, u32 n, u32 bmWords = 0) {
  Work w; size_t o = 0;
  w.first = (u16 *)(base + o); o += pad16((size_t)nFirst * 2);
  w.bm = (u32 *)(base + o); o += pad16((size_t)bmWords * 4);
  w.pre = (u16 *)(base + o); o += pad16((size_t)bmWords * 2);
  w.root = (u16 *)(base + o); o += pad16((size_t)n * 2);
  w.hist = (u32 *)(base + o); w.histWords = (n + 3) / 4;
  return w;
}
__host__ __device__ inline size_t mergeBytes(u32 nRep) {
  return (((size_t)nRep + 15) & ~(size_t)15) + 256 * 8 * 4 + 256 * 4 + 512 * 4 + 16;
}

template <bool IN_LDS, typename T> __device__ __forceinline__ T ld_shared(const T *p) {
  if (IN_LDS) return *p;
  return __hip_atomic_load(p, __ATOMIC_RELAXED, __HIP_MEMORY_SCOPE_AGENT);
}

template <bool IN_LDS>
__device__ __forceinline__ void min_u16(u16 *arr, u32 idx, u32 val) {
  u32 *w = (u32 *)arr + (idx >> 1); const int sh = (idx & 1) * 16;
  u32 old = ld_shared<IN_LDS>(w);
// ... 1590 lines not shown
        p += __longlong_as_double((long long)bits);
      }
    }
  }
  if (lane == 0) blocks[c].pointToMin = p;
}

constexpr int MERGE_THREADS = 256;
constexpr u32 MERGE_SMALL_READS = 4096;
template <bool BIG>
__global__ __launch_bounds__(MERGE_THREADS)
void read_merge_kernel(h10x_block *__restrict__ blocks, const u64 *__restrict__ blockOff, const u32 *__restrict__ nGood,
                       h10x_clushash *__restrict__ clusHash, u32 codeMin) {
  extern __shared__ __align__(16) unsigned char smem[];
  __shared__ u32 changed;
  const u32 c = codeMin + blockIdx.x;
  if (!nGood[c]) return;
  const h10x_block blk = blocks[c];
  const u32 nSub = blk.nSubCluster, nHash = blk.nHash, nRead = blk.nRead;
  if (!nSub) return;
  if ((nRead > MERGE_SMALL_READS) != BIG) return;
  const int tid = threadIdx.x;
  const u32 nRep = nRead < 65536u ? nRead : 65536u;
  h10x_clushash *ch = clusHash + blockOff[c];
  u8 *readRep = (u8 *)smem;
  u32 *adj = (u32 *)(smem + ((nRep + 15) & ~15u));
  u32 *comp = adj + 256 * 8, *newLab = comp + 256;
  constexpr int MERGE_KEEP = 8;
  h10x_clushash keep[MERGE_KEEP];
#pragma unroll
  for (int j = 0; j < MERGE_KEEP; ++j) { const u32 p = tid + j * MERGE_THREADS; keep[j] = ch[p < nHash ? p : nHash - 1]; }
#define H10X_FOR_ENTRIES(...)                                                                                          \
  { _Pragma("unroll") for (int j = 0; j < MERGE_KEEP; ++j) { const u32 p = tid + j * MERGE_THREADS; if (p < nHash) { const h10x_clushash e = keep[j]; __VA_ARGS__ } } \
    for (u32 p = tid + MERGE_KEEP * MERGE_THREADS; p < nHash; p += MERGE_THREADS) { const h10x_clushash e = ch[p]; __VA_ARGS__ } }
  for (u32 i = tid; i < (nRep + 3) / 4; i += MERGE_THREADS) ((u32 *)readRep)[i] = 0;
  for (u32 i = tid; i < 256 * 8; i += MERGE_THREADS) adj[i] = 0;
  comp[tid] = tid;
  __syncthreads();
  H10X_FOR_ENTRIES(
    if (e.subCluster && e.subCluster <= nSub && e.read < nRep) readRep[e.read] = e.subCluster; )
  __syncthreads();
  H10X_FOR_ENTRIES(
    if (e.subCluster && e.subCluster <= nSub && e.read < nRep) {
      const u32 L = e.subCluster, R = readRep[e.read];
      if (R != L) { atomicOr(&adj[L * 8 + (R >> 5)], 1u << (R & 31)); atomicOr(&adj[R * 8 + (L >> 5)], 1u << (L & 31)); }
    } )
  __syncthreads();
  for (int iter = 0; iter < 256; ++iter) {
    if (tid == 0) changed = 0;
    __syncthreads();
    if (tid >= 1 && tid <= (int)nSub) {
      const u32 mine = comp[tid]; u32 m = mine;
      for (int wd = 0; wd < 8; ++wd) { u32 bits = adj[tid * 8 + wd]; while (bits) { const int b = __ffs((int)bits) - 1; bits &= bits - 1; const u32 cR = *(volatile u32 *)&comp[wd * 32 + b]; m = cR < m ? cR : m; } }
      if (m < mine) { atomicMin(&comp[tid], m); changed = 1; }
    }
    __syncthreads();
    if (!changed) break;
    __syncthreads();
  }
  {
    const bool isMin = tid >= 1 && tid <= (int)nSub && comp[tid] == (u32)tid;
    const u64 bal = __ballot(isMin);
    const int lane = tid & (WAVE - 1), wv = tid / WAVE;
    if (lane == 0) newLab[256 + 256 - 4 + wv] = (u32)__popcll(bal);
    __syncthreads();
    u32 before = 0;
    for (int q = 0; q < wv; ++q) before += newLab[256 + 256 - 4 + q];
    newLab[tid] = before + (u32)__popcll(bal & ((2ULL << lane) - 1));
    __syncthreads();
    if (tid == 0) blocks[c].nSubCluster = newLab[nSub];
    u32 mapped = 0;
    if (tid >= 1 && tid <= (int)nSub) mapped = newLab[comp[tid]];
    __syncthreads();
    newLab[256 + tid] = mapped;
    __syncthreads();
  }
  H10X_FOR_ENTRIES(
    const u32 L = e.subCluster;
    if (L && L <= nSub) ch[p].subCluster = (u8)newLab[256 + L]; )
#undef H10X_FOR_ENTRIES
}

__global__ void cluster_classify_kernel(const h10x_block *__restrict__ blocks, const u32 *__restrict__ nGood, const u32 *__restrict__ entries, u32 codeMin, u32 codeMax,
                                        u32 nBlocks , int ranked , u32 hashMinSlots, u32 maxTrRanks, u32 firstCap, u32 bmWords, u32 waves0, size_t budget0, size_t budgetSmall, size_t budgetBig, u32 bigRanks, u32 estDiv ,
                                        u32 *__restrict__ list0, u32 *__restrict__ list1, u32 *__restrict__ list2, u32 *__restrict__ list3,
                                        u32 *__restrict__ listBig , u32 *__restrict__ counts, unsigned long long *__restrict__ work) {
  const u32 c = codeMin + blockIdx.x * blockDim.x + threadIdx.x;
  const int lane = threadIdx.x & (WAVE - 1);
  const u32 n = c < codeMax ? nGood[c] : 0;
  int cls = -1; u32 nRead = 0;
  if (n) {
    nRead = blocks[c].nRead;
    if (ranked == 3) {
      u32 S, S2, nW; bool compact;
      translatedShape(n, waves0, budget0, hashMinSlots, entries[c], nBlocks, firstCap, S, S2, nW, compact);
      if (n > maxTrRanks) cls = 3;
      else if (translatedFits(S, S2, rankedFirstEstimateE(nBlocks, n, entries[c], estDiv), entries[c], nBlocks)) cls = 0;
      else { translatedShape(n, CL_THREADS_HUGE / WAVE, budgetBig, hashMinSlots, entries[c], nBlocks, firstCap, S, S2, nW, compact); cls = S ? 2 : 3; }
    }
    else if (histWaves(ranked ? rankedFirstEstimateE(nBlocks, n, entries[c]) : nBlocks, n, waves0, bmWords, budget0)) cls = 0;
    else if (histWaves(ranked ? rankedFirstEstimate(nBlocks, n) : nBlocks, n, CL_THREADS_HUGE / WAVE, bmWords, budgetBig)) cls = 2;
    else cls = 3;
  }
  if (cls == 0 && n > bigRanks) cls = 1;
  for (int s = 32; s; s >>= 1) nRead = max(nRead, (u32)__shfl_xor((int)nRead, s));
  if (lane == 0 && nRead) atomicMax(&counts[8], nRead);
  {
    u32 n0 = (cls == 0 || cls == 1) ? n : 0u, n2 = cls == 2 ? n : 0u;
    for (int s = 32; s; s >>= 1) { n0 = max(n0, (u32)__shfl_xor((int)n0, s)); n2 = max(n2, (u32)__shfl_xor((int)n2, s)); }
    if (lane == 0) { if (n0) atomicMax(&counts[12], n0); if (n2) atomicMax(&counts[13], n2); }
  }
  if (work) {
    unsigned long long w0 = (cls == 0 || cls == 1) ? (unsigned long long)entries[c] + 64ull * n : 0ull, w2 = cls == 2 ? (unsigned long long)entries[c] + 64ull * n : 0ull;
    for (int s = 32; s; s >>= 1) { w0 += __shfl_xor(w0, s); w2 += __shfl_xor(w2, s); }
    if (lane == 0) { if (w0) atomicAdd(&work[0], w0); if (w2) atomicAdd(&work[1], w2); }
  }
  {
    const u64 bal = __ballot(n > REPLAY_SMALL);
    if (bal) {
      u32 base = 0;
      if (lane == 0) base = atomicAdd(&counts[9], (u32)__popcll(bal));
      base = (u32)__shfl((int)base, 0);
      if (n > REPLAY_SMALL) listBig[base + (u32)__popcll(bal & ((1ULL << lane) - 1))] = c;
    }
  }
  u32 *const lists[4] = {list0, list1, list2, list3};
#pragma unroll
  for (int k = 0; k < 4; ++k) {
    const u64 bal = __ballot(cls == k);
    if (!bal) continue;
    u32 base = 0;
    if (lane == 0) base = atomicAdd(&counts[k], (u32)__popcll(bal));
    base = (u32)__shfl((int)base, 0);
    if (cls == k) lists[k][base + (u32)__popcll(bal & ((1ULL << lane) - 1))] = c;
  }
}

static int cluster_local_range(Ctx *c, int codeMin, int codeMax, int threshold, bool more) {
  hipStream_t st = c->stream;
  const u32 nGlobal = c->sharded ? c->nBlocksGlobal : c->nBlocks;
  c->tstart(T_CLUSTER);
  const u32 span = (u32)(codeMax - codeMin);
  DevBuf<u32> list0, list1, list2, list3, listBig; DevBuf<u64> zeroed; DevBuf<u64> term;
  H10X_HIP(c, list0.alloc(span)); H10X_HIP(c, list1.alloc(span)); H10X_HIP(c, list2.alloc(span)); H10X_HIP(c, list3.alloc(span)); H10X_HIP(c, listBig.alloc(span));
  H10X_HIP(c, zeroed.alloc(8 + 8 + 2)); H10X_HIP(c, term.alloc(c->nEntries));
  H10X_HIP(c, hipMemsetAsync(zeroed.p, 0, (8 + 8 + 2) * 8, st));
  struct { u32 *p; } counts{(u32 *)zeroed.p}; struct { u64 *p; } stats{zeroed.p + 8};
  const size_t budgetSmall = c->optClusterLds > 0 ? (size_t)c->optClusterLds : 80 * 1024 - 1024;
  const size_t budgetBig = c->optClusterLds > 0 ? (size_t)c->optClusterLds : 160 * 1024 - 1024;
  const int threads0 = c->optClusterThreads0 == 512 ? 512 : (c->optClusterThreads0 == 768 ? 768 : 1024);
  const size_t budget0 = c->optClusterLds > 0 ? (size_t)c->optClusterLds : (c->optClusterBudget0 > 0 ? (size_t)c->optClusterBudget0 : budgetSmall);
  const u32 bmWordsAll = (nGlobal + 31) / 32;
  int hashBits = 1; while (hashBits < 32 && (1ull << hashBits) < (unsigned long long)nGlobal) ++hashBits;
  const u32 hashMinSlots = hashBits > 10 ? 4u << (hashBits - 10) : 0u;
  const bool rankedSure = (size_t)bmWordsAll * 6 <= 48 * 1024, rankedTry = !rankedSure && (size_t)bmWordsAll * 6 <= 100 * 1024 && hashBits <= 22;
  int firstMode = (size_t)nGlobal * 2 <= 48 * 1024 ? 0 : (rankedSure || rankedTry ? 1 : (hashBits <= 22 ? 4 : 2));
  if (c->optFirstGlobal == 1) firstMode = 2; else if (c->optFirstGlobal == 2) firstMode = 1;
  else if ((c->optFirstGlobal == 3 || c->optFirstGlobal == 4) && hashBits <= 22) firstMode = 4;
  u32 hStride = 64; while (hStride < c->maxGoodDepth && hStride < (1u << 24)) hStride <<= 1;
  const size_t trSlotCapBytes = (size_t)32 << 20;
  const u32 maxTrRanks = (u32)hmin<size_t>(0xFFFFFFFFu, trSlotCapBytes / ((size_t)hStride * 2));
  const bool packed = c->optTrPacked != 0;
  auto trSlotFor = [&](u32 maxRanks, u32 waves) { return (size_t)hmin<u32>(hmax<u32>(maxRanks, 1u), maxTrRanks) * hStride + 256 + (size_t)waves * TR_QUEUE * 4; };
  const u32 firstCap = c->optFirstCap > 0 ? (u32)c->optFirstCap : 0u;
  u32 hc[14]; u64 hw[2] = {0, 0}; u32 nFirstLds = 0, bmWords = 0;
  for (int attempt = 0; attempt < 2; ++attempt) {
    nFirstLds = firstMode == 0 ? nGlobal : 0;
    bmWords = firstMode == 1 ? bmWordsAll : 0;
    cluster_classify_kernel<<<divUp(span, 256), 256, 0, st>>>(c->blocks.p, c->nGood.p, c->goodEntries.p, (u32)codeMin, (u32)codeMax,
                                                            firstMode == 1 || firstMode >= 3 ? nGlobal : nFirstLds, firstMode == 1 ? 1 : (firstMode == 4 ? 3 : 0), hashMinSlots, maxTrRanks, firstCap,
                                                            bmWords, (u32)threads0 / WAVE, budget0, budgetSmall, budgetBig, c->optBigRanks > 0 ? (u32)c->optBigRanks : c->meanGood + c->meanGood / 2, c->optTrEstDiv > 0 ? (u32)c->optTrEstDiv : 6u,
                                                            list0.p, list1.p, list2.p, list3.p, listBig.p, counts.p, (unsigned long long *)(zeroed.p + 16));
    H10X_TRY(c->readback(hc, counts.p, 56));
    H10X_TRY(c->readback(hw, zeroed.p + 16, 16));
    H10X_TRY(c->syncReadbacks());
    const u32 classified = hc[0] + hc[1] + hc[2] + hc[3];
    if (attempt || !rankedTry || c->optFirstGlobal || firstMode != 1 || hc[3] <= 16 + classified / 200) break;
    firstMode = 4;
    H10X_HIP(c, hipMemsetAsync(counts.p, 0, 16, st));
    H10X_HIP(c, hipMemsetAsync(counts.p + 9, 0, 4, st));
    H10X_HIP(c, hipMemsetAsync(zeroed.p + 16, 0, 16, st));
    H10X_HIP(c, hipMemsetAsync(counts.p + 12, 0, 8, st));
  }
  ClusterArgs a{};
  a.blocks = c->blocks.p; a.blockOff = c->blockOff.p; a.clusHash = c->clusHash.p; a.goodPos = c->goodPos.p; a.nGood = c->nGood.p;
  a.goodRow = c->goodRow.p; a.rows = c->rows.p; a.nBlocks = c->nBlocks; a.threshold = threshold;
  a.segs = c->segs; a.nBlocksFirst = nGlobal; a.rowShift = (u32)c->rowShift;
  if (c->sharded && c->optRowsFakeBase) a.rows = c->rows.p - (size_t)c->optRowsFakeBase;
  a.narrowFirst = (u32)c->optNarrowFirst; a.tpClassT = c->optTrClassT != 0 ? 1u : 0u;
  a.maxGood = c->maxGood; a.stats = stats.p; a.res = term.p; a.entries = c->goodEntries.p;
  a.firstCap = firstCap; a.hashMinSlots = hashMinSlots;
  a.hashBits = (u32)hashBits; a.hStride = hStride;
  const size_t trStride[3] = {trSlotFor(hc[12], (u32)threads0 / WAVE), trSlotFor(hmax<u32>(hc[12], hc[13]), CL_THREADS_HUGE / WAVE), trSlotFor(hmax<u32>(hc[12], hc[13]), CL_THREADS_HUGE / WAVE)};
  DevBuf<u32> ovfA, ovfB; H10X_HIP(c, ovfA.alloc(span)); H10X_HIP(c, ovfB.alloc(span));
  u32 *const ovfCountA = counts.p + 10, *const ovfCountB = counts.p + 11;
  DevBuf<u64> phase;
  if (c->optStamps) { H10X_HIP(c, phase.alloc(8)); H10X_HIP(c, hipMemsetAsync(phase.p, 0, 64, st)); a.phase = phase.p; }
  DevBuf<unsigned char> scratch;
  size_t stride = 0; u32 grid3 = 0;
  if (hc[3]) {
    stride = (workBytes(nGlobal, c->maxGood, CL_THREADS_SMALL / WAVE, 0) + 255) & ~(size_t)255;
    grid3 = hmin<u32>(hc[3], (u32)c->numCU);
    H10X_HIP(c, scratch.alloc(stride * grid3));
    H10X_HIP(c, hipMemsetAsync(scratch.p, 0xFF, stride * grid3, st));
  }
  DevBuf<unsigned char> firstSlots[3];
  const size_t firstStride = (((size_t)nGlobal * 2 + 255) & ~(size_t)255);
  u32 gridOf[3] = {hmin<u32>(hc[0] + hc[1], (u32)c->numCU * (u32)hmax<size_t>(1, (160 * 1024) / (budget0 + 1024))), hmin<u32>(hc[1], (u32)c->numCU * 2), hmin<u32>(hc[2], (u32)c->numCU)};
  u32 secondWind = 0;
  if (firstMode == 4 && gridOf[2] && gridOf[0] >= (u32)c->numCU && hw[0] + hw[1]) {
    const double share2 = 1.25 * (double)hw[1] / (1.25 * (double)hw[1] + (double)hw[0]);
    const u32 cu2 = hmin<u32>((u32)c->numCU > 16 ? (u32)c->numCU - 8 : (u32)c->numCU - 1, hmax<u32>(hmax<u32>(1u, (u32)c->numCU / 8u), (u32)(share2 * c->numCU + 0.5) + 4u));
    gridOf[2] = hmin<u32>(hc[2], cu2);
    gridOf[0] = hmin<u32>(gridOf[0], 2 * (u32)c->numCU);
    secondWind = hc[2] > gridOf[2] ? hmin<u32>(hc[2] - gridOf[2], (u32)c->numCU) : 0u;
  }
  DevBuf<u16> trSlots[3];
  auto trAlloc = [&](int k, u32 &grid) -> int {
    for (;;) {
      if (trSlots[k].alloc(trStride[k] * grid) == hipSuccess) return 0;
      (void)hipGetLastError();
      if (grid <= 1) return c->fail("no device memory for the handle slots of the cluster kernel (%.1f MB per workgroup)", trStride[k] * 2 / 1e6);
      grid = (grid + 1) / 2;
    }
  };
  if (firstMode == 4) for (int k = 0; k < 3; k += 2) if (gridOf[k]) H10X_TRY(trAlloc(k, gridOf[k]));
  if (secondWind) H10X_TRY(trAlloc(1, secondWind));
  if (firstMode == 2) for (int k = 0; k < 3; k += 2) if (gridOf[k]) {
    H10X_HIP(c, firstSlots[k].alloc(firstStride * gridOf[k]));
    H10X_HIP(c, hipMemsetAsync(firstSlots[k].p, 0xFF, firstStride * gridOf[k], st));
  }
  ForkGuard forkGuard(c);
  c->tstart(T_CLUSTER_K);
  H10X_TRY(c->forkStreams(3));
  if (hc[3]) {
    ClusterArgs g = a; g.list = list3.p; g.nList = hc[3]; g.workCounter = counts.p + 7; g.scratch = scratch.p; g.scratchStride = stride;
    cluster_kernel<false, 2, CL_THREADS_SMALL><<<grid3, CL_THREADS_SMALL, 0, c->aux[0]>>>(g);
  }
#define H10X_LAUNCH_ONE(MODE, K, THREADS, BUDGET, GRID, STREAM)                                                                    \
      { H10X_HIP(c, hipFuncSetAttribute((const void *)cluster_kernel<true, MODE, THREADS, K>, hipFuncAttributeMaxDynamicSharedMemorySize, (int)(BUDGET))); \
        cluster_kernel<true, MODE, THREADS, K><<<GRID, THREADS, BUDGET, STREAM>>>(g); }
#define H10X_LAUNCH_LDS(K, THREADS, BUDGET, STREAM, LIST, NLIST, GRID, CNT, OVFCNT, OVF)                                           \
  {                                                                                                                                \
    ClusterArgs g = a; g.list = LIST; g.nList = NLIST; g.workCounter = counts.p + CNT; g.ldsBudget = (u32)(BUDGET);                \
    g.overflow = (OVF); g.overflowCount = (OVFCNT);                                                                                \
    if (firstMode == 0) H10X_LAUNCH_ONE(0, K, THREADS, BUDGET, GRID, STREAM)                                                       \
    else if (firstMode == 1) H10X_LAUNCH_ONE(1, K, THREADS, BUDGET, GRID, STREAM)                                                  \
    else if (firstMode == 4) { g.handles = trSlots[K].p; g.handleStride = trStride[K]; if (packed) H10X_LAUNCH_ONE(5, K, THREADS, BUDGET, GRID, STREAM) else H10X_LAUNCH_ONE(4, K, THREADS, BUDGET, GRID, STREAM) } \
    else { g.scratch = firstSlots[K].p; g.scratchStride = firstStride; H10X_LAUNCH_ONE(2, K, THREADS, BUDGET, GRID, STREAM) }      \
  }
  if (hc[2]) {
    if (!c->startFlags) H10X_HIP(c, hipHostMalloc((void **)&c->startFlags, 1024 * sizeof(u32), hipHostMallocDefault));
    memset(c->startFlags, 0, 1024 * sizeof(u32));
    a.started = (gridOf[2] * 2 <= (u32)c->numCU || secondWind) && gridOf[2] <= 1024 ? c->startFlags : nullptr;
    H10X_LAUNCH_LDS(2, CL_THREADS_HUGE, budgetBig, c->aux[1], list2.p, hc[2], gridOf[2], 6, ovfCountB, ovfB.p)
    if (a.started) {
      const auto t0 = std::chrono::steady_clock::now();
      for (;;) {
        u32 up = 0;
        for (u32 i = 0; i < gridOf[2]; ++i) up += __atomic_load_n(&c->startFlags[i], __ATOMIC_RELAXED) ? 1u : 0u;
        if (up == gridOf[2] || std::chrono::steady_clock::now() - t0 > std::chrono::microseconds(500)) break;
      }
    }
    a.started = nullptr;
  }
  if (hc[0] || hc[1]) {
// ... 32 lines not shown
    if (nB) {
      const u32 grid = hmin<u32>(nB, (u32)c->numCU);
      H10X_HIP(c, scratch2.alloc(firstStride * grid));
      H10X_HIP(c, hipMemsetAsync(scratch2.p, 0xFF, firstStride * grid, st));
      H10X_HIP(c, hipMemsetAsync(counts.p + 7, 0, 4, st));
      ClusterArgs g = a; g.list = ovfB.p; g.nList = nB; g.workCounter = counts.p + 7; g.scratch = scratch2.p; g.scratchStride = firstStride;
      g.ldsBudget = (u32)budgetBig;
      H10X_HIP(c, hipFuncSetAttribute((const void *)cluster_kernel<true, 2, CL_THREADS_HUGE, 3>, hipFuncAttributeMaxDynamicSharedMemorySize, (int)budgetBig));
      cluster_kernel<true, 2, CL_THREADS_HUGE, 3><<<grid, CL_THREADS_HUGE, budgetBig, st>>>(g);
      H10X_HIP(c, hipGetLastError());
    }
  }
#undef H10X_LAUNCH_LDS
#undef H10X_LAUNCH_ONE
  DevBuf<unsigned char> replayScratch;
  {
    if (c->clusterRaw.n != 2 * (size_t)c->nBlocks) { H10X_HIP(c, c->clusterRaw.alloc(2 * (size_t)c->nBlocks)); H10X_HIP(c, hipMemsetAsync(c->clusterRaw.p, 0, 8 * (size_t)c->nBlocks, st)); }
    H10X_HIP(c, hipMemsetAsync(c->clusterRaw.p + 2 * (size_t)codeMin, 0, 8 * (size_t)span, st));
    ReplayArgs ra{}; ra.raw = c->clusterRaw.p; ra.blocks = c->blocks.p; ra.blockOff = c->blockOff.p; ra.clusHash = c->clusHash.p; ra.goodPos = c->goodPos.p; ra.nGood = c->nGood.p;
    ra.res = term.p; ra.codeMin = (u32)codeMin; ra.span = span;
    if (hc[9]) {
      H10X_TRY(c->forkStreams(1));
      ReplayArgs rb = ra; rb.list = listBig.p; rb.span = hc[9];
      const size_t lds = replayBytes(hmin<u32>(REPLAY_MID, c->maxGood));
      H10X_HIP(c, hipFuncSetAttribute((const void *)replay_kernel<true, 1024>, hipFuncAttributeMaxDynamicSharedMemorySize, (int)lds));
      rb.nLo = REPLAY_SMALL; rb.nHi = REPLAY_MID;
      replay_kernel<true, 1024><<<hc[9], 1024, lds, c->aux[0]>>>(rb);
    }
    ra.nLo = 0; ra.nHi = REPLAY_SMALL;
    replay_kernel<true, 256><<<span, 256, replayBytes(hmin<u32>(REPLAY_SMALL, hmax<u32>(c->maxGood, 1))), st>>>(ra);
    ra.list = listBig.p; ra.span = hc[9];
    if (hc[9]) H10X_TRY(c->joinStreams(1));
    if (hc[9] && c->maxGood > REPLAY_MID) {
      const u32 grid = hmin<u32>(hc[9], (u32)c->numCU);
      ra.scratchStride = (replayBytes(c->maxGood) + 255) & ~(size_t)255;
      H10X_HIP(c, replayScratch.alloc(ra.scratchStride * grid));
      ra.scratch = replayScratch.p; ra.nLo = REPLAY_MID; ra.nHi = 0xFFFFFFFFu;
      replay_kernel<false, 1024><<<grid, 1024, 0, st>>>(ra);
    }
    H10X_HIP(c, hipGetLastError());
  }
  H10X_TRY(c->forkStreams(1));
  point_sum_kernel<<<divUp(span, SUM_THREADS / WAVE), SUM_THREADS, 0, c->aux[0]>>>(c->blocks.p, c->blockOff.p, c->nGood.p, (const double *)term.p, (u32)codeMin, (u32)codeMax);
  {
    const size_t ldsSmall = mergeBytes(MERGE_SMALL_READS), ldsBig = mergeBytes(65536);
    read_merge_kernel<false><<<span, MERGE_THREADS, ldsSmall, st>>>(c->blocks.p, c->blockOff.p, c->nGood.p, c->clusHash.p, (u32)codeMin);
    if (hc[8] > MERGE_SMALL_READS) {
      H10X_HIP(c, hipFuncSetAttribute((const void *)read_merge_kernel<true>, hipFuncAttributeMaxDynamicSharedMemorySize, (int)ldsBig));
      read_merge_kernel<true><<<span, MERGE_THREADS, ldsBig, st>>>(c->blocks.p, c->blockOff.p, c->nGood.p, c->clusHash.p, (u32)codeMin);
    }
  }
  H10X_HIP(c, hipGetLastError());
  H10X_TRY(c->faultAt(5));
  H10X_TRY(c->joinStreams(1));
  c->tstop(T_CLUSTER_K);
  u64 hs[8];
  H10X_TRY(c->readback(hs, stats.p, 64));
  H10X_TRY(c->syncReadbacks());
  c->tstop(T_CLUSTER);
  if (c->optStamps) { H10X_HIP(c, hipMemcpy(c->ctr.cluster_phase_ticks, phase.p, 64, hipMemcpyDeviceToHost)); }
  forkGuard.done();
  if (!more) { memset(c->ctr.cluster_main, 0, sizeof c->ctr.cluster_main); memset(c->ctr.cluster_class_counts, 0, sizeof c->ctr.cluster_class_counts);
               c->ctr.sum_good = c->ctr.sum_good_depth = c->ctr.sum_hash_clustered = c->ctr.clustered_codes = c->ctr.cluster_overflow_blocks = 0; }
  for (int k = 0; k < 4; ++k) { c->ctr.cluster_main[k] += hs[4 + k]; hs[k] += hs[4 + k]; }
  c->ctr.sum_good += hs[0]; c->ctr.sum_good_depth += hs[1]; c->ctr.sum_hash_clustered += hs[2]; c->ctr.clustered_codes += span;
  c->ctr.cluster_first_mode = (uint64_t)firstMode; c->ctr.cluster_overflow_blocks += nOverflow;
  for (int k = 0; k < 4; ++k) c->ctr.cluster_class_counts[k] += hc[k];
  return 0;
}

int stageC_readMerge(Ctx *c, u32 code) {
  hipStream_t st = c->stream;
  const size_t ldsSmall = mergeBytes(MERGE_SMALL_READS), ldsBig = mergeBytes(65536);
  read_merge_kernel<false><<<1, MERGE_THREADS, ldsSmall, st>>>(c->blocks.p, c->blockOff.p, c->nGood.p, c->clusHash.p, code);
  H10X_HIP(c, hipFuncSetAttribute((const void *)read_merge_kernel<true>, hipFuncAttributeMaxDynamicSharedMemorySize, (int)ldsBig));
  read_merge_kernel<true><<<1, MERGE_THREADS, ldsBig, st>>>(c->blocks.p, c->blockOff.p, c->nGood.p, c->clusHash.p, code);
  H10X_HIP(c, hipGetLastError());
  return 0;
}

int stageC_cluster(Ctx *c, int codeMin, int codeMax, int threshold) {
  if (!c->haveGood) return c->fail("!! you must set hashDepthRange before cluster");
  if (threshold < 1) return c->fail("clusterThreshold %d must be >= 1 (the reference reads an uninitialised msBest otherwise)", threshold);
  if (c->maxGoodDepth > RES_COUNT_MAX) return c->fail("a hash of the depth range lies in %u barcodes: beyond %u, the limit of this build", c->maxGoodDepth, RES_COUNT_MAX);
  const u32 nGlobal = c->sharded ? c->nBlocksGlobal : c->nBlocks;
  if (!codeMin) codeMin = 1;
  if (!codeMax) codeMax = (int)nGlobal;
  if (codeMin < 0 || codeMax > (int)nGlobal) return c->fail("cluster code range %d..%d outside 1..%u", codeMin, codeMax, nGlobal);
  bool any = false;
  for (int k = 0; k < c->segs.n; ++k) {
    const BlockSeg &sg = c->segs.s[k];
    const long first = (long)sg.localStart + (k == 0 ? 1 : 0);
    long lo = (long)codeMin - (long)sg.globalBase + (long)sg.localStart, hi = (long)codeMax - (long)sg.globalBase + (long)sg.localStart;
    if (lo < first) lo = first;
    if (hi > (long)sg.localStart + (long)sg.count) hi = (long)sg.localStart + (long)sg.count;
    if (hi <= lo) continue;
    H10X_TRY(cluster_local_range(c, (int)lo, (int)hi, threshold, any));
    any = true;
  }
  if (!any) { memset(c->ctr.cluster_class_counts, 0, sizeof c->ctr.cluster_class_counts); memset(c->ctr.cluster_main, 0, sizeof c->ctr.cluster_main);
              c->ctr.sum_good = c->ctr.sum_good_depth = c->ctr.sum_hash_clustered = c->ctr.clustered_codes = c->ctr.cluster_overflow_blocks = 0; }
  return 0;
}

__global__ void split_count_kernel(const h10x_block *__restrict__ oldB, const u64 *__restrict__ oldOff, const h10x_clushash *__restrict__ ch,
                                   u32 nCodes, const u32 *__restrict__ subBefore , SegMap segs,
                                   h10x_block *__restrict__ newB, u32 *__restrict__ newNHash) {
  const u32 i = blockIdx.x; if (i >= nCodes) return;
  const h10x_block ob = oldB[i];
  __shared__ u32 cnt[256];
  for (u32 t = threadIdx.x; t < 256; t += blockDim.x) cnt[t] = 0;
  __syncthreads();
  if (!ob.nSubCluster) {
    if (threadIdx.x == 0) { h10x_block b = ob; b.clusHash = 0; newB[i] = b; newNHash[i] = (i >= 1) ? ob.nHash : 0; }
    return;
  }
  const h10x_clushash *e = ch + oldOff[i];
  for (u32 p = threadIdx.x; p < ob.nHash; p += blockDim.x) atomicAdd(&cnt[e[p].subCluster], 1u);
  __syncthreads();
  const u32 ext = nCodes - 1 + subBefore[i];
  for (u32 j = threadIdx.x; j <= ob.nSubCluster && j < 256; j += blockDim.x) {
    h10x_block b; memset(&b, 0, sizeof b);
    if (j == 0) { b.nRead = ob.nRead; b.nHash = cnt[0]; newB[i] = b; newNHash[i] = cnt[0]; }
    else { b.nHash = cnt[j]; b.clusterParent = segs.globalOf(i) + 1; newB[ext + j] = b; newNHash[ext + j] = cnt[j]; }
  }
}

__global__ void split_move_kernel(const h10x_block *__restrict__ oldB, const u64 *__restrict__ oldOff, const h10x_clushash *__restrict__ ch,
                                  u32 nCodes, const u32 *__restrict__ subBefore, const u64 *__restrict__ readOff ,
                                  u32 *__restrict__ readMap , h10x_block *__restrict__ newB, const u64 *__restrict__ newOff,
                                  h10x_clushash *__restrict__ out) {
  const u32 i = blockIdx.x; if (i >= nCodes) return;
  const h10x_block ob = oldB[i];
  const h10x_clushash *e = ch + oldOff[i];
  if (!ob.nSubCluster) {
    if (i >= 1) for (u32 p = threadIdx.x; p < ob.nHash; p += blockDim.x) out[newOff[i] + p] = e[p];
    return;
  }
  if (threadIdx.x != 0) return;
  __shared__ u32 cursor[256], nReadNew[256];
  for (u32 j = 0; j <= ob.nSubCluster && j < 256; ++j) { cursor[j] = 0; nReadNew[j] = 0; }
  const u32 ext = nCodes - 1 + subBefore[i];
  u32 *rm = readMap + readOff[i];
  for (u32 p = 0; p < ob.nHash; ++p) {
    h10x_clushash c = e[p]; const u32 cl = c.subCluster; c.subCluster = 0;
    if (cl && cl <= ob.nSubCluster) {
      if (!rm[c.read]) rm[c.read] = ++nReadNew[cl];
      c.read = (u16)(rm[c.read] - 1);
      out[newOff[ext + cl] + cursor[cl]++] = c;
    } else out[newOff[i] + cursor[0]++] = c;
  }
  for (u32 j = 1; j <= ob.nSubCluster && j < 256; ++j) newB[ext + j].nRead = nReadNew[j];
}

__global__ void split_aux_kernel(const h10x_block *__restrict__ b, u32 n, u32 *__restrict__ nSub, u32 *__restrict__ nReadP1) {
  const u32 i = blockIdx.x * blockDim.x + threadIdx.x;
  if (i < n) { nSub[i] = b[i].nSubCluster; nReadP1[i] = b[i].nSubCluster ? (b[i].nRead > 65535u ? 65536u : b[i].nRead) + 1 : 0; }
}

int stageC_split(Ctx *c) {
  hipStream_t st = c->stream; PrimTemp pt;
  if (!c->haveState) return c->fail("no hash state loaded: use readFQB or readHash first");
  c->tstart(T_SPLIT);
  const u32 nCodes = c->nBlocks;
  DevBuf<u32> nSub, subBefore, nReadP1; DevBuf<u64> readOff;
  H10X_HIP(c, nSub.alloc((size_t)nCodes + 1)); H10X_HIP(c, subBefore.alloc((size_t)nCodes + 1));
  H10X_HIP(c, nReadP1.alloc((size_t)nCodes + 1)); H10X_HIP(c, readOff.alloc((size_t)nCodes + 1));
// ... 36 lines not shown
```

Baseline: 514.2 million read-pairs/s.

## Defer good-depth stats readback to device, fuse run extraction into scan output

Good-hash statistics (max depth, max and mean good per barcode) are now reduced on the device into a GoodStats buffer. The cluster classify kernel reads them directly, and the host fetches them later alongside other readbacks, which removes a blocking sync in depthRange. Run extraction for packed keys is folded into the rocPRIM inclusive scan through a custom output iterator, so the ordinal array and a separate scatter kernel go away. Smaller changes merge the within and within-depth kernels, skip allocating and zeroing the fallback pointer array when it is unused, and move the overflow counter into an existing buffer. The cost is more complex code and a depth-limit check that now runs later, inside cluster setup.

Result: no change. 512.4 million read-pairs/s (median of 2 runs) (-0.4%).

```diff
diff --git a/hash10x_amd/csrc/common.hpp b/hash10x_amd/csrc/common.hpp
--- a/hash10x_amd/csrc/common.hpp
+++ b/hash10x_amd/csrc/common.hpp
@@ -159,6 +159,7 @@
   u32 rangeHiMax = 0;
   u32 depthBound = 0xFFFFFFFFu;
   u32 maxGoodDepth = 0, maxGood = 0, meanGood = 0;
+  DevBuf<u32> goodStats; bool goodStatsOnHost = true; u32 goodStatsDiv = 0;
 
   DevBuf<u32> cribCount[2];
   DevBuf<u64> cribFirst[2];
diff --git a/hash10x_amd/csrc/h10x_api.hip b/hash10x_amd/csrc/h10x_api.hip
--- a/hash10x_amd/csrc/h10x_api.hip
+++ b/hash10x_amd/csrc/h10x_api.hip
@@ -218,7 +218,7 @@
 
 static void reset_state(Ctx &c) {
   c.haveState = false; c.haveRange = false; c.haveGood = false; c.rangeMin = c.rangeMax = 0; c.depthBound = 0xFFFFFFFFu; c.rangeHiMax = 0;
-  c.within.release(); c.goodPos.release(); c.nGood.release(); c.goodEntries.release(); c.goodRow.release();
+  c.within.release(); c.goodStats.release(); c.goodStatsOnHost = true; c.goodPos.release(); c.nGood.release(); c.goodEntries.release(); c.goodRow.release();
   c.hashIndex.release(); c.hashValue.release(); c.hashDepth.release(); c.rowStart.release(); c.rows.release();
   c.blocks.release(); c.blockOff.release(); c.clusHash.release(); c.clusterRaw.release();
   c.hashNumber = 1; c.nBlocks = 0; c.nEntries = 0; c.nRecords = 0; c.maxBlockHashes = 0xFFFFFFFFu;
diff --git a/hash10x_amd/csrc/prim.hip b/hash10x_amd/csrc/prim.hip
--- a/hash10x_amd/csrc/prim.hip
+++ b/hash10x_amd/csrc/prim.hip
@@ -1,5 +1,6 @@
 #include "prim.hpp"
 #include <thread>
+#include <iterator>
 #include <rocprim/rocprim.hpp>
 
 namespace h10x {
@@ -26,6 +27,36 @@
 int prim_run_ordinals_u64(Ctx *c, PrimTemp &t, const u64 *key, int cb, u32 *ord, size_t n) {
   auto flags = rocprim::make_transform_iterator(rocprim::counting_iterator<size_t>(0), RunHead{key, n, cb});
   PRIM_TWO_PHASE(c, t, rocprim::exclusive_scan(tmp, bytes, flags, ord, (u32)0, n + 1, rocprim::plus<u32>(), c->stream));
+  return 0;
+}
+struct RunSink { const u64 *key; size_t n; int cb; u32 cap; Val16 *dVal; u32 *dFirst, *rows, *nRuns; };
+struct RunSinkRef {
+  RunSink s; size_t i;
+  __device__ void operator=(u32 inc) const {
+    const u64 k = s.key[i], q = k >> s.cb;
+    const u32 code = (u32)(k & (((u64)1 << s.cb) - 1)), d = inc - 1;
+    s.rows[i] = code;
+    const bool head = i == 0 || (s.key[i - 1] >> s.cb) != q, tail = i + 1 == s.n || (s.key[i + 1] >> s.cb) != q;
+    if (d < s.cap) {
+      if (head) { s.dVal[d].a = q; s.dVal[d].b = (u32)i; s.dFirst[d] = code; }
+      if (tail) s.dVal[d].c = (u32)i + 1;
+    }
+    if (i + 1 == s.n) *s.nRuns = inc;
+  }
+};
+struct RunSinkIter {
+  using iterator_category = std::random_access_iterator_tag; using value_type = u32; using difference_type = std::ptrdiff_t; using pointer = void; using reference = RunSinkRef;
+  RunSink s; size_t i;
+  __host__ __device__ RunSinkIter operator+(difference_type d) const { return RunSinkIter{s, i + (size_t)d}; }
+  __host__ __device__ RunSinkIter &operator+=(difference_type d) { i += (size_t)d; return *this; }
+  __host__ __device__ RunSinkRef operator[](difference_type d) const { return RunSinkRef{s, i + (size_t)d}; }
+  __host__ __device__ RunSinkRef operator*() const { return RunSinkRef{s, i}; }
+};
+int prim_run_extract_packed_u64(Ctx *c, PrimTemp &t, const u64 *key, int cb, size_t n, u32 cap, Val16 *dVal, u32 *dFirst, u32 *rows, u32 *nRuns) {
+  if (!n) return 0;
+  auto flags = rocprim::make_transform_iterator(rocprim::counting_iterator<size_t>(0), RunHead{key, n, cb});
+  RunSinkIter out{RunSink{key, n, cb, cap, dVal, dFirst, rows, nRuns}, 0};
+  PRIM_TWO_PHASE(c, t, rocprim::inclusive_scan(tmp, bytes, flags, out, n, rocprim::plus<u32>(), c->stream));
   return 0;
 }
 int prim_exclusive_scan_u32_u64(Ctx *c, PrimTemp &t, const u32 *in, u64 *out, size_t n) {
diff --git a/hash10x_amd/csrc/prim.hpp b/hash10x_amd/csrc/prim.hpp
--- a/hash10x_amd/csrc/prim.hpp
+++ b/hash10x_amd/csrc/prim.hpp
@@ -13,6 +13,7 @@
 int prim_sort_pairs_u32_u32(Ctx *c, PrimTemp &t, const u32 *kin, u32 *kout, const u32 *vin, u32 *vout, size_t n, int beginBit, int endBit);
 int prim_sort_keys_u64(Ctx *c, PrimTemp &t, const u64 *kin, u64 *kout, size_t n, int beginBit, int endBit);
 struct Val16 { u64 a; u32 b, c; };
+int prim_run_extract_packed_u64(Ctx *c, PrimTemp &t, const u64 *key, int cb, size_t n, u32 cap, Val16 *dVal, u32 *dFirst, u32 *rows, u32 *nRuns);
 int prim_sort_pairs_u32_v16(Ctx *c, PrimTemp &t, const u32 *kin, u32 *kout, const Val16 *vin, Val16 *vout, size_t n, int beginBit, int endBit);
 int prim_seg_sort_keys_u64(Ctx *c, PrimTemp &t, const u64 *kin, u64 *kout, u32 n, u32 nSeg, const u32 *begin, const u32 *end, int beginBit, int endBit);
 int prim_seg_sort_keys_u32(Ctx *c, PrimTemp &t, const u32 *kin, u32 *kout, u32 n, u32 nSeg, const u32 *begin, const u32 *end, int beginBit, int endBit);
diff --git a/hash10x_amd/csrc/stage_a.hip b/hash10x_amd/csrc/stage_a.hip
--- a/hash10x_amd/csrc/stage_a.hip
+++ b/hash10x_amd/csrc/stage_a.hip
@@ -377,7 +377,7 @@
   for (u32 c = blockIdx.x + 1; c < nBlocks; c += gridDim.x) {
     const u32 n = nHash[c]; if (!n) continue;
     const u64 *sh; const u32 *sr;
-    if (fb[c].hash) { sh = fb[c].hash; sr = fb[c].read; } else { sh = stHash + capOff[c]; sr = stRead + capOff[c]; }
+    if (fb && fb[c].hash) { sh = fb[c].hash; sr = fb[c].read; } else { sh = stHash + capOff[c]; sr = stRead + capOff[c]; }
     const u64 o = blockOff[c];
     if (codeBits) for (u32 i = threadIdx.x; i < n; i += blockDim.x) { entHash[o + i] = (((sh[i] >> keyShift) * keyInv) << codeBits) | c; entRead[o + i] = sr[i]; }
     else for (u32 i = threadIdx.x; i < n; i += blockDim.x) { entHash[o + i] = (sh[i] >> keyShift) * keyInv; entCode[o + i] = c; entRead[o + i] = sr[i]; }
@@ -517,8 +517,9 @@
   const int packedOK = (2 * k + 16 <= 64) ? 1 : 0;
   DevBuf<u32> slots, list0, list1, list2, listF, counts, nHash;
   H10X_HIP(c, slots.alloc(nBlocks)); H10X_HIP(c, list0.alloc(nBlocks)); H10X_HIP(c, list1.alloc(nBlocks)); H10X_HIP(c, list2.alloc(nBlocks));
-  H10X_HIP(c, listF.alloc(nBlocks)); H10X_HIP(c, counts.alloc(4)); H10X_HIP(c, nHash.alloc((size_t)nBlocks + 1));
-  H10X_HIP(c, hipMemsetAsync(counts.p, 0, 16, st));
+  H10X_HIP(c, listF.alloc(nBlocks)); H10X_HIP(c, counts.alloc(8)); H10X_HIP(c, nHash.alloc((size_t)nBlocks + 1));
+  u32 *const nOverflow = counts.p + 4;
+  H10X_HIP(c, hipMemsetAsync(counts.p, 0, 32, st));
   H10X_HIP(c, hipMemsetAsync(nHash.p, 0, ((size_t)nBlocks + 1) * 4, st));
   classify_kernel<<<divUp(nBlocks, 256), 256, 0, st>>>(startRec.p, nBlocks, c->blocks.p, slots.p, maxSlots, packedOK,
                                                       list0.p, list1.p, list2.p, listF.p, counts.p, hashLast ? 1 : 0);
@@ -560,8 +561,7 @@
   forkGuard.done();
   c->tstop(T_MOSH);
 
-  DevBuf<u32> nOverflow; H10X_HIP(c, nOverflow.alloc(1)); H10X_HIP(c, hipMemsetAsync(nOverflow.p, 0, 4, st));
-  count_overflow_kernel<<<divUp(nBlocks, 256), 256, 0, st>>>(nHash.p, nBlocks, nOverflow.p);
+  count_overflow_kernel<<<divUp(nBlocks, 256), 256, 0, st>>>(nHash.p, nBlocks, nOverflow);
   H10X_HIP(c, c->blockOff.alloc((size_t)nBlocks + 1));
   H10X_TRY(prim_exclusive_scan_u32_u64(c, pt, nHash.p, c->blockOff.p, (size_t)nBlocks + 1));
   u64 H = 0, lastStart = 0; u32 hOverflow = 0, hMaxHash = 0xFFFFFFFFu;
@@ -570,7 +570,7 @@
   H10X_TRY(c->readback(&hMaxHash, dMaxHash.p, 4));
   H10X_TRY(c->readback(&H, c->blockOff.p + nBlocks, 8));
   H10X_TRY(c->readback(&lastStart, startRec.p + (nBlocks - 1), 8));
-  H10X_TRY(c->readback(&hOverflow, nOverflow.p, 4));
+  H10X_TRY(c->readback(&hOverflow, nOverflow, 4));
   H10X_TRY(c->syncReadbacks());
   const bool anyFallback = hc[3] || hOverflow;
   std::vector<u32> hNHash, hListF(hc[3]);
@@ -624,9 +624,9 @@
   }
 
   c->tstart(T_COMPACT);
-  DevBuf<SrcPtr> dFb; H10X_HIP(c, dFb.alloc(nBlocks));
-  if (hFb.empty()) H10X_HIP(c, hipMemsetAsync(dFb.p, 0, (size_t)nBlocks * sizeof(SrcPtr), st));
-  else {
+  DevBuf<SrcPtr> dFb;
+  if (!hFb.empty()) {
+    H10X_HIP(c, dFb.alloc(nBlocks));
     H10X_HIP(c, hipMemcpyAsync(dFb.p, hFb.data(), (size_t)nBlocks * sizeof(SrcPtr), hipMemcpyHostToDevice, st));
     H10X_TRY(prim_exclusive_scan_u32_u64(c, pt, nHash.p, c->blockOff.p, (size_t)nBlocks + 1));
     H10X_HIP(c, hipMemcpyAsync(&H, c->blockOff.p + nBlocks, 8, hipMemcpyDeviceToHost, st));
diff --git a/hash10x_amd/csrc/stage_b.hip b/hash10x_amd/csrc/stage_b.hip
--- a/hash10x_amd/csrc/stage_b.hip
+++ b/hash10x_amd/csrc/stage_b.hip
@@ -15,19 +15,6 @@
   for (; i < n; i += stride) if (ord[i + 1] != ord[i]) {
     const u32 d = ord[i];
     dHash[d] = sHash[i]; dFirst[d] = sCode[i]; segStart[d] = (u32)i; iota[d] = d;
-  }
-}
-__global__ void seg_scatter_packed_kernel(const u64 *__restrict__ sKey, int cb,
-                                          const u32 *__restrict__ ord, u64 n, Val16 *__restrict__ dVal, u32 *__restrict__ dFirst, u32 *__restrict__ rows) {
-  u64 i = (u64)blockIdx.x * blockDim.x + threadIdx.x;
-  const u64 stride = (u64)gridDim.x * blockDim.x;
-  const u64 cmask = ((u64)1 << cb) - 1;
-  for (; i < n; i += stride) {
-    const u64 k = sKey[i]; const u32 code = (u32)(k & cmask);
-    rows[i] = code;
-    const u32 d = ord[i], d1 = ord[i + 1];
-    if (d1 != d) { dVal[d].a = k >> cb; dVal[d].b = (u32)i; dFirst[d] = code; }
-    if (i + 1 == n || ord[i + 2] != d1) dVal[d1 - 1].c = (u32)i + 1;
   }
 }
 __global__ void assign_index_v16_kernel(const Val16 *__restrict__ val, u32 U, u64 w , u64 *__restrict__ hashValue, u32 *__restrict__ hashDepth,
@@ -397,18 +384,25 @@
   c->tstart(T_RANK);
   u32 U = 0;
   DevBuf<u64> dHash; DevBuf<u32> dFirst, segStart, iota, order, dFirstSorted; DevBuf<Val16> dVal, dValSorted;
-  {
+  const u64 indexLimit = (tableSize >> 2) - 2;
+  if (cb) {
+    const u32 cap = (u32)hmin<u64>(H, indexLimit);
+    DevBuf<u32> nRuns;
+    H10X_HIP(c, dVal.alloc(cap)); H10X_HIP(c, dFirst.alloc(cap)); H10X_HIP(c, nRuns.alloc(1));
+    H10X_TRY(prim_run_extract_packed_u64(c, pt, sHash.p, cb, H, cap, dVal.p, dFirst.p, sCode.p, nRuns.p));
+    if (H) { H10X_TRY(c->readback(&U, nRuns.p, 4)); H10X_TRY(c->syncReadbacks()); }
+    if ((u64)U + 1 > indexLimit) return c->fail("hashTableSize is too small");
+    H10X_HIP(c, dFirstSorted.alloc(U)); H10X_HIP(c, dValSorted.alloc(U));
+  } else {
     DevBuf<u32> ord;
-    H10X_HIP(c, ord.alloc(H + 2));
+    H10X_HIP(c, ord.alloc(H + 1));
     H10X_TRY(prim_run_ordinals_u64(c, pt, sHash.p, cb, ord.p, H));
     H10X_TRY(c->readback(&U, ord.p + H, 4));
     H10X_TRY(c->syncReadbacks());
-    if ((u64)U + 1 > (tableSize >> 2) - 2) return c->fail("hashTableSize is too small");
+    if ((u64)U + 1 > indexLimit) return c->fail("hashTableSize is too small");
     H10X_HIP(c, dFirst.alloc(U)); H10X_HIP(c, dFirstSorted.alloc(U));
-    if (cb) { H10X_HIP(c, dVal.alloc(U)); H10X_HIP(c, dValSorted.alloc(U)); }
-    else { H10X_HIP(c, dHash.alloc(U)); H10X_HIP(c, segStart.alloc((size_t)U + 1)); H10X_HIP(c, iota.alloc(U)); H10X_HIP(c, order.alloc(U)); }
-    if (H && cb) seg_scatter_packed_kernel<<<gH, 256, 0, st>>>(sHash.p, cb, ord.p, H, dVal.p, dFirst.p, sCode.p);
-    else if (H) {
+    H10X_HIP(c, dHash.alloc(U)); H10X_HIP(c, segStart.alloc((size_t)U + 1)); H10X_HIP(c, iota.alloc(U)); H10X_HIP(c, order.alloc(U));
+    if (H) {
       seg_scatter_kernel<<<gH, 256, 0, st>>>(sHash.p, sCode.p, ord.p, H, dHash.p, dFirst.p, segStart.p, iota.p);
       H10X_HIP(c, hipMemsetD32Async((hipDeviceptr_t)(segStart.p + U), (int)(u32)H, 1, st));
     }
diff --git a/hash10x_amd/csrc/stage_c.hip b/hash10x_amd/csrc/stage_c.hip
--- a/hash10x_amd/csrc/stage_c.hip
+++ b/hash10x_amd/csrc/stage_c.hip
@@ -14,19 +14,40 @@
 constexpr int ROWS_IN_FLIGHT = 4;
 constexpr int RCHUNK = 4;
 
-__global__ void within_kernel(const u32 *__restrict__ depth, u32 hashNumber, int lo, int hi, u8 *__restrict__ within) {
-  const u32 i = blockIdx.x * blockDim.x + threadIdx.x;
-  if (i >= hashNumber) return;
-  const int n = (int)depth[i];
-  if (n >= lo && n < hi) within[i] = 1;
-}
-__global__ void within_depth_kernel(const u32 *__restrict__ depth, const u8 *__restrict__ within, u32 hashNumber, u32 *__restrict__ out,
-                                    const u64 *__restrict__ rowStart, u32 rowShift, u64 *__restrict__ rowInfo ) {
-  const u32 i = blockIdx.x * blockDim.x + threadIdx.x;
-  if (i < hashNumber) {
-    const u32 wd = within[i] ? depth[i] + 1 : 0;
-    out[i] = wd; if (rowInfo) rowInfo[i] = (u64)(u32)(rowStart[i] >> rowShift) | ((u64)wd << 32);
-  }
+struct GoodStats { u32 maxDepth1, maxGood; unsigned long long sumGood; };
+static_assert(sizeof(GoodStats) == 16, "GoodStats is cleared and read back as four words");
+__host__ __device__ inline u32 trListStride(u32 maxGoodDepth) { u32 h = 64; while (h < maxGoodDepth && h < (1u << 24)) h <<= 1; return h; }
+__host__ __device__ inline u32 trMaxRanks(u32 hStride) { const size_t r = ((size_t)32 << 20) / ((size_t)hStride * 2); return r > 0xFFFFFFFFu ? 0xFFFFFFFFu : (u32)r; }
+
+__global__ __launch_bounds__(256)
+void within_depth_kernel(const u32 *__restrict__ depth, u32 hashNumber, int set, int lo, int hi, u8 *__restrict__ within, int derive, u32 *__restrict__ wdepth ,
+                         const u64 *__restrict__ rowStart, u32 rowShift, u64 *__restrict__ rowInfo ,
+                         GoodStats *__restrict__ stats) {
+  __shared__ u32 sMax;
+  if (threadIdx.x == 0) sMax = 0;
+  __syncthreads();
+  u32 m = 0;
+  const u64 stride = (u64)gridDim.x * blockDim.x;
+  for (u64 i = (u64)blockIdx.x * blockDim.x + threadIdx.x; i < hashNumber; i += stride) {
+    const u32 d = depth[i];
+    bool in;
+    if (set) {
+      const bool hit = (int)d >= lo && (int)d < hi;
+      if (set == 1) { within[i] = hit ? 1 : 0; in = hit; }
+      else { in = hit || within[i] != 0; if (hit) within[i] = 1; }
+    } else in = within[i] != 0;
+    if (derive) {
+      const u32 wd = in ? d + 1 : 0;
+      m = wd > m ? wd : m;
+      if (wdepth) wdepth[i] = wd;
+      if (rowInfo) rowInfo[i] = (u64)(u32)(rowStart[i] >> rowShift) | ((u64)wd << 32);
+    }
+  }
+  if (!derive) return;
+  for (int sft = 32; sft; sft >>= 1) { const u32 o = (u32)__shfl_xor((int)m, sft); m = o > m ? o : m; }
+  if ((threadIdx.x & (WAVE - 1)) == 0 && m) atomicMax(&sMax, m);
+  __syncthreads();
+  if (threadIdx.x == 0 && sMax > *(volatile u32 *)&stats->maxDepth1) atomicMax(&stats->maxDepth1, sMax);
 }
 
 template <typename KT>
@@ -121,9 +142,37 @@
   }
 }
 
+constexpr u32 GOOD_STATS_WG = 64;
+__global__ __launch_bounds__(256)
+void good_stats_kernel(const u32 *__restrict__ nGood, u32 nBlocks, GoodStats *__restrict__ stats) {
+  __shared__ u32 sMax; __shared__ unsigned long long sSum;
+  if (threadIdx.x == 0) { sMax = 0; sSum = 0; }
+  __syncthreads();
+  u32 m = 0; unsigned long long t = 0;
+  for (u32 c = blockIdx.x * blockDim.x + threadIdx.x; c < nBlocks; c += gridDim.x * blockDim.x) { const u32 n = nGood[c]; m = n > m ? n : m; t += n; }
+  for (int sft = 32; sft; sft >>= 1) { const u32 o = (u32)__shfl_xor((int)m, sft); m = o > m ? o : m; t += __shfl_xor(t, sft); }
+  if ((threadIdx.x & (WAVE - 1)) == 0 && t) { atomicMax(&sMax, m); atomicAdd(&sSum, t); }
+  __syncthreads();
+  if (threadIdx.x == 0 && sSum) { atomicMax(&stats->maxGood, sMax); atomicAdd(&stats->sumGood, sSum); }
+}
+
 __global__ void good_rows_kernel(const h10x_clushash *__restrict__ ch, const u64 *__restrict__ blockOff, const u32 *__restrict__ nGood, const u16 *__restrict__ goodPos, u32 nBlocks,
                                  const u32 *__restrict__ hashDepth, const u64 *__restrict__ rowStart, u32 rowShift, u64 *__restrict__ goodRow);
 static int bitsForC(u64 maxValue) { int b = 1; while (b < 64 && (maxValue >> b)) ++b; return b; }
+
+static void goodStatsSet(Ctx *c, const GoodStats &g) {
+  c->maxGoodDepth = g.maxDepth1 ? g.maxDepth1 - 1 : 0;
+  c->maxGood = g.maxGood; c->meanGood = c->goodStatsDiv ? (u32)(g.sumGood / c->goodStatsDiv) : 0;
+  c->goodStatsOnHost = true;
+}
+static int goodStatsHost(Ctx *c) {
+  if (c->goodStatsOnHost) return 0;
+  GoodStats g;
+  H10X_TRY(c->readback(&g, c->goodStats.p, sizeof g));
+  H10X_TRY(c->syncReadbacks());
+  goodStatsSet(c, g);
+  return 0;
+}
 
 int stageC_depthRange(Ctx *c, int lo, int hi) {
   hipStream_t st = c->stream; PrimTemp pt;
@@ -131,25 +180,31 @@
   c->haveGood = false;
   c->tstart(T_GOOD);
   const u32 U1 = c->hashNumber; const u32 nBlocks = c->nBlocks; const u64 H = c->nEntries;
+  int set = 0;
   if (!(c->haveRange && lo == c->rangeMin && hi == c->rangeMax)) {
-    if (!c->haveRange) { H10X_HIP(c, c->within.alloc(U1)); H10X_HIP(c, hipMemsetAsync(c->within.p, 0, U1, st)); }
-    within_kernel<<<divUp(U1, 256), 256, 0, st>>>(c->hashDepth.p, U1, lo, hi, c->within.p);
+    set = c->haveRange ? 2 : 1;
+    if (!c->haveRange) H10X_HIP(c, c->within.alloc(U1));
     c->haveRange = true; c->rangeMin = lo; c->rangeMax = hi;
     if (hi > 0 && (u32)hi > c->rangeHiMax) c->rangeHiMax = (u32)hi;
   }
+  const unsigned gU = divUp(U1, 256);
+  H10X_HIP(c, c->goodStats.alloc(sizeof(GoodStats) / 4));
+  GoodStats *const stats = (GoodStats *)c->goodStats.p;
+  H10X_HIP(c, hipMemsetAsync(stats, 0, sizeof(GoodStats), st));
+  c->goodStatsOnHost = false; c->goodStatsDiv = nBlocks > 1 ? nBlocks - 1 : 0;
   XGuard xGuard(c);
-  if (c->sharded) { c->tstop(T_GOOD); H10X_TRY(shard_exchangeRows(c)); c->tstart(T_GOOD); }
-  DevBuf<u64> key, keyS; DevBuf<u32> key32, keyS32, off32, segEnd, wdepth, red;
-  H10X_HIP(c, off32.alloc((size_t)nBlocks + 1));
-  H10X_HIP(c, segEnd.alloc(nBlocks)); H10X_HIP(c, wdepth.alloc(U1)); H10X_HIP(c, red.alloc(2));
+  if (c->sharded) {
+    if (set) within_depth_kernel<<<gU, 256, 0, st>>>(c->hashDepth.p, U1, set, lo, hi, c->within.p, 0, nullptr, nullptr, 0, nullptr, stats);
+    set = 0;
+    c->tstop(T_GOOD); H10X_TRY(shard_exchangeRows(c)); c->tstart(T_GOOD);
+  }
   H10X_HIP(c, c->nGood.alloc(nBlocks)); H10X_HIP(c, c->goodPos.alloc(H)); H10X_HIP(c, c->goodEntries.alloc(nBlocks)); H10X_HIP(c, c->goodRow.alloc(H));
   const u32 goodDepthBound = hmin<u32>(c->depthBound, c->rangeHiMax ? c->rangeHiMax - 1 : 0);
   const bool narrow = goodDepthBound <= 65535u;
   const bool byBlocks = narrow && c->maxBlockHashes <= BLOCK_SORT_MAX;
-  DevBuf<u64> rowInfo; if (byBlocks) H10X_HIP(c, rowInfo.alloc(U1));
-  within_depth_kernel<<<divUp(U1, 256), 256, 0, st>>>(c->hashDepth.p, c->within.p, U1, wdepth.p, c->rowStart.p, (u32)c->rowShift, rowInfo.p);
-  H10X_TRY(prim_reduce_max_u32(c, pt, wdepth.p, red.p, U1));
   if (byBlocks) {
+    DevBuf<u64> rowInfo; H10X_HIP(c, rowInfo.alloc(U1));
+    within_depth_kernel<<<gU, 256, 0, st>>>(c->hashDepth.p, U1, set, lo, hi, c->within.p, 1, nullptr, c->rowStart.p, (u32)c->rowShift, rowInfo.p, stats);
     int db = 1; while (db < 16 && (goodDepthBound >> db)) ++db;
     const int sortBits = db + 1;
     DevBuf<u32> lists, counts;
@@ -168,34 +223,31 @@
     H10X_TRY(c->faultAt(3));
     if (side) H10X_TRY(c->joinStreams(side));
     forkGuard.done();
-  }
-  else if (narrow) { H10X_HIP(c, key32.alloc(H)); H10X_HIP(c, keyS32.alloc(H)); } else { H10X_HIP(c, key.alloc(H)); H10X_HIP(c, keyS.alloc(H)); }
-  if (byBlocks) {}
-  else if (narrow) good_keys_kernel<u32><<<hmin<u32>(nBlocks, 16384), 256, 0, st>>>(c->clusHash.p, c->blockOff.p, c->blocks.p, nBlocks, wdepth.p,
-                                                                             key32.p, c->nGood.p, segEnd.p, c->goodEntries.p);
-  else good_keys_kernel<u64><<<hmin<u32>(nBlocks, 16384), 256, 0, st>>>(c->clusHash.p, c->blockOff.p, c->blocks.p, nBlocks, wdepth.p,
-                                                                      key.p, c->nGood.p, segEnd.p, c->goodEntries.p);
-  H10X_TRY(prim_reduce_max_u32(c, pt, c->nGood.p, red.p + 1, nBlocks));
-  DevBuf<u64> redSum; H10X_HIP(c, redSum.alloc(1));
-  H10X_TRY(prim_reduce_sum_u32_u64(c, pt, c->nGood.p, redSum.p, nBlocks));
-  u32 hr[2]; u64 sumGood = 0;
-  H10X_TRY(c->readback(hr, red.p, 8));
-  H10X_TRY(c->readback(&sumGood, redSum.p, 8));
-  H10X_TRY(c->syncReadbacks());
-  hr[0] = hr[0] ? hr[0] - 1 : 0;
-  c->maxGoodDepth = hr[0]; c->maxGood = hr[1]; c->meanGood = nBlocks > 1 ? (u32)(sumGood / (nBlocks - 1)) : 0;
-  offsets32c_kernel<<<divUp((u64)nBlocks + 1, 256), 256, 0, st>>>(c->blockOff.p, nBlocks + 1, off32.p);
-  if (H && !byBlocks) {
-    if (narrow) {
-      H10X_TRY(prim_seg_sort_keys_u32(c, pt, key32.p, keyS32.p, (u32)H, nBlocks, off32.p, segEnd.p, 0, 16 + bitsForC(hr[0])));
-      good_pos_kernel<u32><<<(unsigned)hmin<u64>(divUp(H, 256), 65535u * 2), 256, 0, st>>>(keyS32.p, H, c->goodPos.p);
-    } else {
-      H10X_TRY(prim_seg_sort_keys_u64(c, pt, key.p, keyS.p, (u32)H, nBlocks, off32.p, segEnd.p, 0, 16 + bitsForC(hr[0])));
-      good_pos_kernel<u64><<<(unsigned)hmin<u64>(divUp(H, 256), 65535u * 2), 256, 0, st>>>(keyS.p, H, c->goodPos.p);
-    }
-  }
-  if (!byBlocks && nBlocks) good_rows_kernel<<<hmin<u32>(nBlocks, 65535u * 4), 256, 0, st>>>(c->clusHash.p, c->blockOff.p, c->nGood.p, c->goodPos.p, nBlocks, c->hashDepth.p, c->rowStart.p,
-                                                                                           (u32)c->rowShift, c->goodRow.p);
+    good_stats_kernel<<<hmin<u32>(divUp(nBlocks, 256), GOOD_STATS_WG), 256, 0, st>>>(c->nGood.p, nBlocks, stats);
+  } else {
+    DevBuf<u64> key, keyS; DevBuf<u32> key32, keyS32, off32, segEnd, wdepth;
+    H10X_HIP(c, off32.alloc((size_t)nBlocks + 1)); H10X_HIP(c, segEnd.alloc(nBlocks)); H10X_HIP(c, wdepth.alloc(U1));
+    within_depth_kernel<<<gU, 256, 0, st>>>(c->hashDepth.p, U1, set, lo, hi, c->within.p, 1, wdepth.p, nullptr, 0, nullptr, stats);
+    if (narrow) { H10X_HIP(c, key32.alloc(H)); H10X_HIP(c, keyS32.alloc(H)); } else { H10X_HIP(c, key.alloc(H)); H10X_HIP(c, keyS.alloc(H)); }
+    if (narrow) good_keys_kernel<u32><<<hmin<u32>(nBlocks, 16384), 256, 0, st>>>(c->clusHash.p, c->blockOff.p, c->blocks.p, nBlocks, wdepth.p,
+                                                                            key32.p, c->nGood.p, segEnd.p, c->goodEntries.p);
+    else good_keys_kernel<u64><<<hmin<u32>(nBlocks, 16384), 256, 0, st>>>(c->clusHash.p, c->blockOff.p, c->blocks.p, nBlocks, wdepth.p,
+                                                                        key.p, c->nGood.p, segEnd.p, c->goodEntries.p);
+    good_stats_kernel<<<hmin<u32>(divUp(nBlocks, 256), GOOD_STATS_WG), 256, 0, st>>>(c->nGood.p, nBlocks, stats);
+    H10X_TRY(goodStatsHost(c));
+    offsets32c_kernel<<<divUp((u64)nBlocks + 1, 256), 256, 0, st>>>(c->blockOff.p, nBlocks + 1, off32.p);
+    if (H) {
+      if (narrow) {
+        H10X_TRY(prim_seg_sort_keys_u32(c, pt, key32.p, keyS32.p, (u32)H, nBlocks, off32.p, segEnd.p, 0, 16 + bitsForC(c->maxGoodDepth)));
+        good_pos_kernel<u32><<<(unsigned)hmin<u64>(divUp(H, 256), 65535u * 2), 256, 0, st>>>(keyS32.p, H, c->goodPos.p);
+      } else {
+        H10X_TRY(prim_seg_sort_keys_u64(c, pt, key.p, keyS.p, (u32)H, nBlocks, off32.p, segEnd.p, 0, 16 + bitsForC(c->maxGoodDepth)));
+        good_pos_kernel<u64><<<(unsigned)hmin<u64>(divUp(H, 256), 65535u * 2), 256, 0, st>>>(keyS.p, H, c->goodPos.p);
+      }
+    }
+    if (nBlocks) good_rows_kernel<<<hmin<u32>(nBlocks, 65535u * 4), 256, 0, st>>>(c->clusHash.p, c->blockOff.p, c->nGood.p, c->goodPos.p, nBlocks, c->hashDepth.p, c->rowStart.p,
+                                                                                (u32)c->rowShift, c->goodRow.p);
+  }
   H10X_HIP(c, hipGetLastError());
   H10X_TRY(c->xJoin());
   c->haveGood = true;
@@ -1952,13 +2004,16 @@
 }
 
 __global__ void cluster_classify_kernel(const h10x_block *__restrict__ blocks, const u32 *__restrict__ nGood, const u32 *__restrict__ entries, u32 codeMin, u32 codeMax,
-                                        u32 nBlocks , int ranked , u32 hashMinSlots, u32 maxTrRanks, u32 firstCap, u32 bmWords, u32 waves0, size_t budget0, size_t budgetSmall, size_t budgetBig, u32 bigRanks, u32 estDiv ,
+                                        u32 nBlocks , int ranked , u32 hashMinSlots,
+                                        const GoodStats *__restrict__ goodStats , u32 meanDiv, u32 bigRanksOpt , u32 firstCap, u32 bmWords, u32 waves0, size_t budget0, size_t budgetSmall, size_t budgetBig, u32 estDiv ,
                                         u32 *__restrict__ list0, u32 *__restrict__ list1, u32 *__restrict__ list2, u32 *__restrict__ list3,
                                         u32 *__restrict__ listBig , u32 *__restrict__ counts, unsigned long long *__restrict__ work) {
   const u32 c = codeMin + blockIdx.x * blockDim.x + threadIdx.x;
   const int lane = threadIdx.x & (WAVE - 1);
   const u32 n = c < codeMax ? nGood[c] : 0;
   int cls = -1; u32 nRead = 0;
+  const u32 maxTrRanks = trMaxRanks(trListStride(goodStats->maxDepth1 ? goodStats->maxDepth1 - 1 : 0));
+  const u32 meanGood = meanDiv ? (u32)(goodStats->sumGood / meanDiv) : 0, bigRanks = bigRanksOpt ? bigRanksOpt : meanGood + meanGood / 2;
   if (n) {
     nRead = blocks[c].nRead;
     if (ranked == 3) {
@@ -2027,9 +2082,7 @@
   int firstMode = (size_t)nGlobal * 2 <= 48 * 1024 ? 0 : (rankedSure || rankedTry ? 1 : (hashBits <= 22 ? 4 : 2));
   if (c->optFirstGlobal == 1) firstMode = 2; else if (c->optFirstGlobal == 2) firstMode = 1;
   else if ((c->optFirstGlobal == 3 || c->optFirstGlobal == 4) && hashBits <= 22) firstMode = 4;
-  u32 hStride = 64; while (hStride < c->maxGoodDepth && hStride < (1u << 24)) hStride <<= 1;
-  const size_t trSlotCapBytes = (size_t)32 << 20;
-  const u32 maxTrRanks = (u32)hmin<size_t>(0xFFFFFFFFu, trSlotCapBytes / ((size_t)hStride * 2));
+  u32 hStride = 0, maxTrRanks = 0;
   const bool packed = c->optTrPacked != 0;
   auto trSlotFor = [&](u32 maxRanks, u32 waves) { return (size_t)hmin<u32>(hmax<u32>(maxRanks, 1u), maxTrRanks) * hStride + 256 + (size_t)waves * TR_QUEUE * 4; };
   const u32 firstCap = c->optFirstCap > 0 ? (u32)c->optFirstCap : 0u;
@@ -2038,12 +2091,16 @@
     nFirstLds = firstMode == 0 ? nGlobal : 0;
     bmWords = firstMode == 1 ? bmWordsAll : 0;
     cluster_classify_kernel<<<divUp(span, 256), 256, 0, st>>>(c->blocks.p, c->nGood.p, c->goodEntries.p, (u32)codeMin, (u32)codeMax,
-                                                            firstMode == 1 || firstMode >= 3 ? nGlobal : nFirstLds, firstMode == 1 ? 1 : (firstMode == 4 ? 3 : 0), hashMinSlots, maxTrRanks, firstCap,
-                                                            bmWords, (u32)threads0 / WAVE, budget0, budgetSmall, budgetBig, c->optBigRanks > 0 ? (u32)c->optBigRanks : c->meanGood + c->meanGood / 2, c->optTrEstDiv > 0 ? (u32)c->optTrEstDiv : 6u,
+                                                            firstMode == 1 || firstMode >= 3 ? nGlobal : nFirstLds, firstMode == 1 ? 1 : (firstMode == 4 ? 3 : 0), hashMinSlots,
+                                                            (const GoodStats *)c->goodStats.p, c->goodStatsDiv, c->optBigRanks > 0 ? (u32)c->optBigRanks : 0u, firstCap,
+                                                            bmWords, (u32)threads0 / WAVE, budget0, budgetSmall, budgetBig, c->optTrEstDiv > 0 ? (u32)c->optTrEstDiv : 6u,
                                                             list0.p, list1.p, list2.p, list3.p, listBig.p, counts.p, (unsigned long long *)(zeroed.p + 16));
     H10X_TRY(c->readback(hc, counts.p, 56));
     H10X_TRY(c->readback(hw, zeroed.p + 16, 16));
+    GoodStats gs; const bool fetch = !c->goodStatsOnHost;
+    if (fetch) H10X_TRY(c->readback(&gs, c->goodStats.p, sizeof gs));
     H10X_TRY(c->syncReadbacks());
+    if (fetch) goodStatsSet(c, gs);
     const u32 classified = hc[0] + hc[1] + hc[2] + hc[3];
     if (attempt || !rankedTry || c->optFirstGlobal || firstMode != 1 || hc[3] <= 16 + classified / 200) break;
     firstMode = 4;
@@ -2052,6 +2109,8 @@
     H10X_HIP(c, hipMemsetAsync(zeroed.p + 16, 0, 16, st));
     H10X_HIP(c, hipMemsetAsync(counts.p + 12, 0, 8, st));
   }
+  if (c->maxGoodDepth > RES_COUNT_MAX) return c->fail("a hash of the depth range lies in %u barcodes: beyond %u, the limit of this build", c->maxGoodDepth, RES_COUNT_MAX);
+  hStride = trListStride(c->maxGoodDepth); maxTrRanks = trMaxRanks(hStride);
   ClusterArgs a{};
   a.blocks = c->blocks.p; a.blockOff = c->blockOff.p; a.clusHash = c->clusHash.p; a.goodPos = c->goodPos.p; a.nGood = c->nGood.p;
   a.goodRow = c->goodRow.p; a.rows = c->rows.p; a.nBlocks = c->nBlocks; a.threshold = threshold;
@@ -2250,7 +2309,6 @@
 int stageC_cluster(Ctx *c, int codeMin, int codeMax, int threshold) {
   if (!c->haveGood) return c->fail("!! you must set hashDepthRange before cluster");
   if (threshold < 1) return c->fail("clusterThreshold %d must be >= 1 (the reference reads an uninitialised msBest otherwise)", threshold);
-  if (c->maxGoodDepth > RES_COUNT_MAX) return c->fail("a hash of the depth range lies in %u barcodes: beyond %u, the limit of this build", c->maxGoodDepth, RES_COUNT_MAX);
   const u32 nGlobal = c->sharded ? c->nBlocksGlobal : c->nBlocks;
   if (!codeMin) codeMin = 1;
   if (!codeMax) codeMax = (int)nGlobal;
```
